# suhrig/arriba

Measured on AMD Instinct MI355X. Metric: chimeric reads/s end-to-end (BAM->fusions.tsv), synthetic, higher is better.
Workload: dtype int32

## Files before the change

arriba_amd/csrc/device/agpu_ingest.hip:

```cpp
#include <hip/hip_runtime.h>
#include <algorithm>
#include <cstring>
#include <string>
#include <vector>
#include <rocprim/rocprim.hpp>
#include "agpu_context.hpp"
#include "ingest_core.hpp"
#include "device_utils.hpp"
#include "shard_host.hpp"
#include "crc32_core.hpp"
#include "inflate_fast_core.hpp"

using namespace agpu;
namespace agpu { extern thread_local bool g_inside_ingest_finish; }

namespace {

const int BLOCK = 256;
inline unsigned int grid_for(uint64_t n, int block = BLOCK) { return (unsigned int) ((n + block - 1) / block); }

enum { IC_ACTIVE = 0, IC_MAPPED_READS = 1, IC_MISSING_HI = 2, IC_BROKEN = 3, IC_MALFORMED = 4, IC_CHIMERIC = 5, IC_COLLISION = 6, IC_MISMATCH = 7, IC_UNSORTED = 8, IC_MAX_NAME = 9,
       IC_MAX_READ_LENGTH = 10, IC_STRAND_COUNT = 11, IC_STRAND_MATCHING = 12, IC_RUNS_UNSORTED = 13, IC_QNAME_COMMA = 14, IC_COUNT = 16 };

#define HIP_CHECK(call) do { hipError_t e_ = (call); if (e_ != hipSuccess) { set_last_error(std::string(#call) + ": " + hipGetErrorString(e_)); return AGPU_ERR_DEVICE; } } while (0)
#define ALLOC(buffer, bytes) do { if (!(buffer).allocate(bytes)) { set_last_error("hipMalloc failed (" #buffer ")"); return AGPU_ERR_NO_MEMORY; } } while (0)
#define TRY(call) do { int s_ = (call); if (s_ != AGPU_OK) return s_; } while (0)


__global__ void __launch_bounds__(BLOCK) bgzf_unwrap_kernel(const uint8_t* raw, const agpu_bgzf_block* blocks, uint8_t* stream) {
	const agpu_bgzf_block block = blocks[blockIdx.x];
	const uint8_t* source = raw + block.raw_offset + block.payload_offset;
	uint8_t* target = stream + block.stream_offset;
	const uint32_t size = block.payload_size;
	uint32_t head = (uint32_t) ((4 - ((uintptr_t) target & 3)) & 3);
	if (head > size) head = size;
	if (threadIdx.x < head) target[threadIdx.x] = source[threadIdx.x];
	const uint32_t words = (size - head) / 4;
	for (uint32_t w = threadIdx.x; w < words; w += BLOCK) *(uint32_t*) (target + head + 4 * (size_t) w) = load_u32(source + head + 4 * (size_t) w);
	const uint32_t tail = head + 4 * words;
	if (threadIdx.x < size - tail) target[tail + threadIdx.x] = source[tail + threadIdx.x];
}

template <int LANES> __global__ void __launch_bounds__(LANES) bgzf_inflate_tokens_kernel(const uint8_t* raw, const agpu_bgzf_block* blocks, uint32_t n_blocks, uint8_t* stream, uint8_t* spill,
                                                                                        unsigned long long* notes, uint32_t* note_count, int* status, unsigned int* failures) {
	__shared__ InflateFastTables tables[LANES];
	const uint32_t b = blockIdx.x * LANES + threadIdx.x;
	if (b >= n_blocks) return;
	const agpu_bgzf_block block = blocks[b];
	const bool partial = block.skip != 0 || block.keep != block.isize;
	uint8_t* target = partial ? spill + (b == 0 ? 0 : 65536) : stream + block.stream_offset;
	uint32_t noted = 0;
	const int result = block.isize > 65536 ? (int) INFLATE_OUTPUT_OVERRUN
	                 : inflate_tokens(raw + block.raw_offset + block.payload_offset, block.payload_size, target, block.isize, notes + (size_t) b * INFLATE_MATCH_CAPACITY, INFLATE_MATCH_CAPACITY, noted, tables[threadIdx.x]);
	note_count[b] = noted; status[b] = result;
	if (result != INFLATE_OK && result != INFLATE_RETRY) atomicAdd(failures, 1u);
}

__global__ void __launch_bounds__(BLOCK) bgzf_inflate_resolve_kernel(const agpu_bgzf_block* blocks, uint32_t n_blocks, uint8_t* stream, uint8_t* spill, const unsigned long long* notes, const uint32_t* note_count, const int* status) {
	const uint32_t b = blockIdx.x * (BLOCK / 64) + (threadIdx.x >> 6), lane = threadIdx.x & 63;
	if (b >= n_blocks || status[b] != INFLATE_OK) return;
	const agpu_bgzf_block block = blocks[b];
	const bool partial = block.skip != 0 || block.keep != block.isize;
	uint8_t* target = partial ? spill + (b == 0 ? 0 : 65536) : stream + block.stream_offset;
	const unsigned long long* mine = notes + (size_t) b * INFLATE_MATCH_CAPACITY;
	const uint32_t n = note_count[b];
	for (uint32_t base = 0; base < n; base += 64) {
		const unsigned long long note = base + lane < n ? mine[base + lane] : 0ull;
		const uint32_t position = inflate_note_position(note), length = inflate_note_length(note), distance = inflate_note_distance(note);
		bool pending = base + lane < n;
		while (true) {
			const unsigned long long waiting = __ballot(pending);
			if (waiting == 0) break;
			const uint32_t frontier = (uint32_t) __shfl((int) position, __ffsll((unsigned long long) waiting) - 1);
			if (pending && inflate_match_is_ready(position, length, distance, frontier)) { inflate_copy_match(target, position, length, distance); pending = false; }
			__builtin_amdgcn_fence(__ATOMIC_SEQ_CST, "workgroup");
		}
	}
	if (partial) for (uint32_t k = lane; k < block.keep; k += 64) stream[block.stream_offset + k] = target[block.skip + k];
}

__global__ void __launch_bounds__(64, 3) bgzf_inflate_kernel(const uint8_t* raw, const agpu_bgzf_block* blocks, uint8_t* stream, uint8_t* spill, int* status, int* verdict, unsigned int* failures) {
	__shared__ InflateShared shared;
	if (status != nullptr && status[blockIdx.x] != INFLATE_RETRY) return;
	const agpu_bgzf_block block = blocks[blockIdx.x];
	const bool partial = block.skip != 0 || block.keep != block.isize;
	uint8_t* target = partial ? spill + (blockIdx.x == 0 ? 0 : 65536) : stream + block.stream_offset;
	auto sync = [] () { __syncthreads(); };
	auto broadcast = [] (uint32_t value) { return (uint32_t) __builtin_amdgcn_readfirstlane((int) value); };
	const int result = inflate_block(raw + block.raw_offset + block.payload_offset, block.payload_size, target, block.isize, shared, threadIdx.x, 64u, sync, broadcast);
	if (verdict != nullptr && threadIdx.x == 0) verdict[blockIdx.x] = result;
	if (result != INFLATE_OK) { if (threadIdx.x == 0) atomicAdd(failures, 1u); return; }
	if (partial) {
		__syncthreads();
		for (uint32_t k = threadIdx.x; k < block.keep; k += 64) stream[block.stream_offset + k] = __hip_atomic_load(&target[block.skip + k], __ATOMIC_RELAXED, __HIP_MEMORY_SCOPE_AGENT);
	}
}


__global__ void segment_guess_kernel(const uint8_t* bytes, uint64_t size, uint64_t base, uint64_t segment_begin, uint64_t n_segments, uint32_t n_targets, uint64_t* first, uint64_t* end, uint32_t* count) {
	const uint64_t s = segment_begin + blockIdx.x * (uint64_t) BLOCK + threadIdx.x;
	if (s < n_segments) guess_segment(bytes, size, base, s, n_targets, first, end, count);
}

__global__ void segment_check_kernel(const uint64_t* first, const uint64_t* end, uint64_t segment_begin, uint64_t n_segments, uint8_t* mismatch, uint32_t* mismatches) {
	__shared__ uint32_t block_sum;
	uint32_t mine = 0;
	for (uint64_t s = segment_begin + blockIdx.x * (uint64_t) BLOCK + threadIdx.x; s < n_segments; s += gridDim.x * (uint64_t) BLOCK) {
		const bool bad = s > 0 && first[s] != end[s - 1];
		mismatch[s] = bad;
		mine += bad;
	}
	block_tally(mine, mismatches, &block_sum);
}

__global__ void segment_repair_kernel(const uint8_t* bytes, uint64_t size, uint64_t base, uint64_t segment_begin, uint64_t n_segments, const uint8_t* mismatch, const uint64_t* previous_end, uint64_t* first, uint64_t* end, uint32_t* count) {
	const uint64_t s = segment_begin + blockIdx.x * (uint64_t) BLOCK + threadIdx.x;
	if (s < n_segments) repair_segment_run(bytes, size, base, n_segments, s, mismatch, previous_end, first, end, count);
}

__global__ void segment_emit_kernel(const uint8_t* bytes, uint64_t size, uint64_t base, uint64_t segment_begin, uint64_t n_segments, const uint64_t* first, const uint32_t* record_base, uint64_t* record_offset) {
	const uint64_t s = segment_begin + blockIdx.x * (uint64_t) BLOCK + threadIdx.x;
	if (s >= n_segments) return;
	const uint64_t begin = base + s * SEGMENT_BYTES, segment_end = (begin + SEGMENT_BYTES < size) ? begin + SEGMENT_BYTES : size;
	uint32_t n = 0;
	walk_segment(bytes, size, first[s], segment_end, n, record_offset + record_base[s]);
}


const uint32_t PARSE_WINDOW = 16384;
__global__ void __launch_bounds__(BLOCK) record_parse_kernel(IngestStream in, GenomeView genome, uint64_t seed, uint64_t record_begin, uint64_t* keys, uint8_t* bits, int32_t* hit_index, uint32_t* counters) {
	__shared__ uint32_t sums[4];
	__shared__ __attribute__((aligned(16))) uint8_t staged[BLOCK / 64][PARSE_WINDOW + 64];
	const uint32_t wave = threadIdx.x / 64, lane = threadIdx.x % 64;
	uint8_t* window = staged[wave];
	uint32_t active = 0, mapped = 0, missing = 0, broken = 0;
	for (uint64_t base = record_begin + ((uint64_t) blockIdx.x * (BLOCK / 64) + wave) * 64; base < in.n_records; base += (uint64_t) gridDim.x * BLOCK) {
		const uint64_t r = base + lane;
		const uint64_t piece_begin = in.record_offset[base] & ~15ull, piece_end = base + 64 < in.n_records ? in.record_offset[base + 64] : in.size;
		const bool in_lds = piece_end > piece_begin && piece_end - piece_begin <= PARSE_WINDOW;
		if (in_lds) {
			for (uint64_t at = piece_begin + 16 * lane; at < piece_end; at += 16 * 64) *(uint4*) (window + (at - piece_begin)) = *(const uint4*) (in.bytes + at);
			__builtin_amdgcn_fence(__ATOMIC_RELEASE, "workgroup"); __builtin_amdgcn_wave_barrier(); __builtin_amdgcn_fence(__ATOMIC_ACQUIRE, "workgroup");
		}
		if (r < in.n_records) {
			const uint64_t offset = in.record_offset[r];
			const uint8_t* p = in.bytes + offset;
			uint32_t block_size = load_u32(p);
			if (in_lds && offset + 4 + (uint64_t) block_size <= piece_end && offset + 36 <= piece_end) { p = window + (offset - piece_begin); block_size = load_u32(p); }
			uint64_t key = ~0ull;
			uint8_t status = RECORD_SKIPPED;
			int32_t hit = HIT_INDEX_UNKNOWN;
			if (!record_sizes_ok(p + 4, block_size)) { status = RECORD_BROKEN; ++broken; }
			else {
				const Rec record = load_record_at(in, p);
				if (!((record.flag & BAMF_UNMAP) || ((record.flag & BAMF_PAIRED) && (record.flag & BAMF_MUNMAP)))) {
					const AuxTags tags = scan_aux(record.aux, record.end);
					if (!tags.has_hi && (record.flag & BAMF_SECONDARY)) { status = RECORD_MISSING_HI; ++missing; }
					else if (record.contig < 0) { status = RECORD_BROKEN; ++broken; }
					else {
						status = RECORD_ACTIVE | (tags.has_sa ? RECORD_HAS_SA : 0);
						key = name_key(record, tags.has_hi ? tags.hi : 1, seed);
						hit = hit_index_to_keep(tags);
						++active;
						if (!(record.flag & BAMF_SUPPLEMENTARY) && (genome.contig_bits[record.contig] & CBIT_INTERESTING)) ++mapped;
					}
				}
			}
			keys[r] = key;
			bits[r] = status;
			hit_index[r] = hit;
		}
		__builtin_amdgcn_fence(__ATOMIC_RELEASE, "workgroup"); __builtin_amdgcn_wave_barrier();
	}
	block_tally(active, &counters[IC_ACTIVE], &sums[0]);
	block_tally(mapped, &counters[IC_MAPPED_READS], &sums[1]);
	block_tally(missing, &counters[IC_MISSING_HI], &sums[2]);
	block_tally(broken, &counters[IC_BROKEN], &sums[3]);
}

__global__ void group_head_kernel(const uint64_t* sorted_keys, uint64_t n_active, uint8_t* head) {
	const uint64_t p = blockIdx.x * (uint64_t) BLOCK + threadIdx.x;
	if (p < n_active) head[p] = p == 0 || sorted_keys[p] != sorted_keys[p - 1];
}
__global__ void group_first_flag_kernel(const uint32_t* sorted_records, const uint32_t* group_start, uint32_t n_groups, uint8_t* first_flags) {
	const uint32_t g = blockIdx.x * BLOCK + threadIdx.x;
	if (g < n_groups) first_flags[sorted_records[group_start[g]]] = 1;
}
__global__ void group_rank_kernel(const uint32_t* sorted_records, const uint32_t* group_start, uint32_t n_groups, uint64_t n_active, const uint32_t* stream_rank, uint32_t* group_first, uint32_t* group_begin, uint32_t* group_count) {
	const uint32_t g = blockIdx.x * BLOCK + threadIdx.x;
	if (g >= n_groups) return;
	const uint32_t begin = group_start[g], first = sorted_records[begin], t = stream_rank[first];
	group_first[t] = first; group_begin[t] = begin; group_count[t] = (uint32_t) ((g + 1 < n_groups ? (uint64_t) group_start[g + 1] : n_active) - begin);
}
__global__ void group_names_kernel(IngestStream in, const uint32_t* sorted_records, const uint32_t* group_begin, const uint32_t* group_count, uint32_t first_group, uint32_t n_groups, uint32_t* counters) {
	const uint32_t t = first_group + blockIdx.x * BLOCK + threadIdx.x;
	if (t >= n_groups || group_count[t] < 2) return;
	const uint32_t* records = sorted_records + group_begin[t];
	const Rec a = load_record(in, records[0]);
	const int64_t hit_a = hit_index_of(in, records[0], a);
	for (uint32_t k = 1; k < group_count[t]; ++k) {
		const Rec b = load_record(in, records[k]);
		if (!same_name(a, hit_a, b, hit_index_of(in, records[k], b))) { atomicOr(&counters[IC_COLLISION], 1u); return; }
	}
}


__global__ void window_carry_kernel(uint32_t* record_base, uint64_t segment_begin, uint64_t segment_end, const uint32_t* records_before) {
	const uint64_t s = segment_begin + blockIdx.x * (uint64_t) BLOCK + threadIdx.x;
	if (s <= segment_end) record_base[s] += *records_before;
}
__global__ void window_summary_kernel(const uint32_t* record_base, const uint64_t* end, uint64_t segment_end, uint32_t* records_before, uint32_t* words) {
	*records_before = record_base[segment_end];
	words[1] = record_base[segment_end];
	const uint64_t last_end = end[segment_end - 1];
	words[4] = (uint32_t) last_end; words[5] = (uint32_t) (last_end >> 32);
}
struct RecordIsActive { __host__ __device__ bool operator()(uint8_t bits) const { return (bits & RECORD_STATUS_MASK) == RECORD_ACTIVE; } };
__global__ void run_head_kernel(const uint64_t* keys, const uint32_t* active_records, uint64_t begin, uint64_t end, uint8_t* head) {
	const uint64_t i = begin + blockIdx.x * (uint64_t) BLOCK + threadIdx.x;
	if (i < end) head[i] = i == 0 || keys[active_records[i]] != keys[active_records[i - 1]];
}
__global__ void run_close_kernel(const uint32_t* active_records, const uint32_t* run_begin, uint32_t first_group, uint32_t n_groups, uint32_t n_runs, uint64_t active_total, uint32_t* group_first, uint32_t* group_count) {
	const uint32_t g = first_group + blockIdx.x * BLOCK + threadIdx.x;
	if (g >= n_groups) return;
	const uint32_t begin = run_begin[g];
	group_first[g] = active_records[begin];
	group_count[g] = (uint32_t) ((g + 1 < n_runs ? (uint64_t) run_begin[g + 1] : active_total) - begin);
}
__global__ void run_key_kernel(const uint64_t* keys, const uint32_t* group_first, uint32_t n_groups, uint64_t* out) {
	const uint32_t g = blockIdx.x * BLOCK + threadIdx.x;
	if (g < n_groups) out[g] = keys[group_first[g]];
}
__global__ void run_repeat_kernel(const uint64_t* sorted_keys, uint32_t n_groups, uint32_t* repeats) {
	__shared__ uint32_t block_sum;
	uint32_t mine = 0;
	for (uint64_t g = blockIdx.x * (uint64_t) BLOCK + threadIdx.x; g < n_groups; g += gridDim.x * (uint64_t) BLOCK) mine += g > 0 && sorted_keys[g] == sorted_keys[g - 1];
	block_tally(mine, repeats, &block_sum);
}

struct ViralCounter {
	unsigned long long* counts;
	__device__ void operator()(uint32_t contig) { atomicAdd(&counts[contig], 1ull); }
};

#ifndef AGPU_REPLAY_WAVES
#define AGPU_REPLAY_WAVES 0
#endif
#ifndef AGPU_PACK_WAVES
#define AGPU_PACK_WAVES 0
#endif
#if AGPU_REPLAY_WAVES > 0
#define AGPU_REPLAY_OCCUPANCY __attribute__((amdgpu_waves_per_eu(AGPU_REPLAY_WAVES, AGPU_REPLAY_WAVES)))
#else
#define AGPU_REPLAY_OCCUPANCY
#endif
#if AGPU_PACK_WAVES > 0
#define AGPU_PACK_OCCUPANCY __attribute__((amdgpu_waves_per_eu(AGPU_PACK_WAVES, AGPU_PACK_WAVES)))
#else
#define AGPU_PACK_OCCUPANCY
#endif
template <bool RUNS> __global__ void __launch_bounds__(BLOCK) AGPU_REPLAY_OCCUPANCY group_replay_kernel(IngestContext ctx, const uint32_t* sorted_records, const uint32_t* group_begin, const uint32_t* group_count, uint32_t first_group, uint32_t n_groups,
                                                             FragmentPlan* plain, TandemPlan* itd, uint8_t* valid, FragmentSizes* sizes, unsigned long long* viral_counts, uint32_t* qname_differs, uint32_t* counters) {
	__shared__ uint32_t sums[2];
	GroupTally tally; tally.malformed = 0; tally.chimeric = 0; tally.collision = 0;
	const uint32_t g = first_group + blockIdx.x * BLOCK + threadIdx.x;
	if (g < n_groups) {
		const uint32_t begin = group_begin[g];
		const uint32_t n_records = group_count[g];
		const Rec representative = load_record(ctx.stream, sorted_records[begin]);
		const int64_t hit = hit_index_of(ctx.stream, sorted_records[begin], representative);
		const uint32_t length = qname_length(representative);
		if (RUNS) {
			if (find_byte(representative.name, length, ',') < length) atomicOr(&counters[IC_QNAME_COMMA], 1u);
			if (g == 0) qname_differs[0] = 0;
			else {
				const uint32_t record_before = sorted_records[group_begin[g - 1]];
				const Rec run_before = load_record(ctx.stream, record_before);
				const uint32_t length_before = qname_length(run_before), shorter = length < length_before ? length : length_before, different = first_difference(run_before.name, representative.name, shorter);
				qname_differs[g] = length != length_before || different < shorter;
				bool unsorted;
				if (different < shorter) unsorted = run_before.name[different] > representative.name[different];
				else unsorted = compare_names(fragment_name(run_before, hit_index_of(ctx.stream, record_before, run_before), false, length_before), fragment_name(representative, hit, false, length)) >= 0;
				if (unsorted) atomicOr(&counters[IC_RUNS_UNSORTED], 1u);
			}
		}
		FragmentPlan plain_plan; TandemPlan itd_plan;
		ViralCounter viral = { viral_counts };
		replay_group(ctx, sorted_records + begin, n_records, plain_plan, itd_plan, tally, viral, RUNS ? &representative : nullptr, length, hit);
		if (tally.collision) atomicOr(&counters[IC_COLLISION], 1u);
		Fragment3 fragment;
		AGPU_NOUNROLL for (uint32_t entry = 0; entry < 2; ++entry) {
			const FragmentPlan& plan = entry ? itd_plan.plan : plain_plan;
			bool ok = false;
			if (plan.count > 0) {
				ok = normalize_plan(ctx.stream, plan, entry ? &itd_plan.tandem : nullptr, fragment);
				if (!ok) tally.malformed++;
			}
			valid[2 * (size_t) g + entry] = ok;
			FragmentSizes mine; mine.cigar_words = 0; mine.sequence_bytes = 0; mine.name_length = 0;
			if (ok) { if (entry) itd[g] = itd_plan; else plain[g] = plain_plan; fragment_sizes(fragment, representative, hit, entry, mine, length); }
			sizes[2 * (size_t) g + entry] = mine;
		}
	}
	block_tally(tally.malformed, &counters[IC_MALFORMED], &sums[0]);
	block_tally(tally.chimeric, &counters[IC_CHIMERIC], &sums[1]);
}


__device__ FragmentName name_of(const IngestStream& in, const uint32_t* group_first, uint32_t ref, Rec& storage) {
	storage = load_record(in, group_first[ref >> 1]);
	return fragment_name(storage, hit_index_of(in, group_first[ref >> 1], storage), ref & 1);
}

__global__ void name_order_check_kernel(IngestStream in, const uint32_t* group_first, const uint32_t* order, uint64_t n, uint32_t* counters) {
	__shared__ uint32_t block_max;
	if (threadIdx.x == 0) block_max = 0;
	__syncthreads();
	const uint64_t i = blockIdx.x * (uint64_t) BLOCK + threadIdx.x;
	if (i < n) {
		Rec storage_a, storage_b;
		const FragmentName mine = name_of(in, group_first, order[i], storage_a);
		atomicMax(&block_max, name_length(mine));
		if (i > 0) {
			const FragmentName before = name_of(in, group_first, order[i - 1], storage_b);
			if (compare_names(before, mine) >= 0) atomicOr(&counters[IC_UNSORTED], 1u);
		}
	}
	__syncthreads();
	if (threadIdx.x == 0 && block_max) atomicMax(&counters[IC_MAX_NAME], block_max);
}

__global__ void run_itd_order_kernel(IngestStream in, const uint32_t* group_first, const uint8_t* valid, uint32_t first_group, uint32_t n_groups, uint32_t* counters) {
	const uint32_t g = first_group + blockIdx.x * BLOCK + threadIdx.x;
	if (g >= n_groups || g == 0 || !valid[2 * (size_t) (g - 1) + 1]) return;
	Rec storage_a, storage_b;
	const FragmentName mine = name_of(in, group_first, 2 * g, storage_b);
	const FragmentName before = name_of(in, group_first, 2 * (g - 1) + 1, storage_a);
	if (compare_names(before, mine) >= 0) atomicOr(&counters[IC_RUNS_UNSORTED], 1u);
}

__global__ void name_chunk_kernel(IngestStream in, const uint32_t* group_first, const uint32_t* order, uint64_t n, uint32_t chunk, uint64_t* keys) {
	const uint64_t i = blockIdx.x * (uint64_t) BLOCK + threadIdx.x;
	if (i >= n) return;
	Rec storage;
	keys[i] = name_chunk(name_of(in, group_first, order[i], storage), chunk);
}


__global__ void fragment_layout_kernel(IngestStream in, const uint32_t* group_first, const uint32_t* order, uint64_t n, const FragmentSizes* sizes, const uint32_t* qname_run ,
                                       uint32_t* cigar_words, uint32_t* sequence_bytes, uint32_t* name_lengths, uint32_t* new_group) {
	const uint64_t i = blockIdx.x * (uint64_t) BLOCK + threadIdx.x;
	if (i > n) return;
	if (i == n) { cigar_words[i] = 0; sequence_bytes[i] = 0; name_lengths[i] = 0; return; }
	const uint32_t ref = order[i];
	const FragmentSizes mine = sizes[ref];
	cigar_words[i] = mine.cigar_words; sequence_bytes[i] = mine.sequence_bytes; name_lengths[i] = mine.name_length;
	uint32_t differs = 0;
	if (i > 0 && qname_run != nullptr) differs = qname_run[ref >> 1] != qname_run[order[i - 1] >> 1];
	else if (i > 0) {
		const Rec a = load_record(in, group_first[ref >> 1]), b = load_record(in, group_first[order[i - 1] >> 1]);
		const uint32_t length = qname_length(a);
		differs = length != qname_length(b);
		for (uint32_t k = 0; k < length && !differs; ++k) differs = a.name[k] != b.name[k];
	}
	new_group[i] = differs;
}

__global__ void __launch_bounds__(BLOCK) AGPU_PACK_OCCUPANCY fragment_pack_kernel(IngestStream in, const uint32_t* group_first, const uint32_t* order, uint64_t n, const FragmentPlan* plain, const TandemPlan* itd,
                                                              const uint64_t* cigar_base, const uint64_t* sequence_base, const uint64_t* name_base, const uint32_t* group_id, PackTarget out, uint32_t* counters) {
	__shared__ uint32_t block_max;
	if (threadIdx.x == 0) block_max = 0;
	__syncthreads();
	const uint64_t i = blockIdx.x * (uint64_t) BLOCK + threadIdx.x;
	if (i == n) out.name_offset[n] = name_base[n];
	if (i < n) {
		const uint32_t ref = order[i], g = ref >> 1;
		const bool is_itd = ref & 1;
		Fragment3 f;
		normalize_plan(in, is_itd ? itd[g].plan : plain[g], is_itd ? &itd[g].tandem : nullptr, f);
		Rec storage;
		const FragmentName name = name_of(in, group_first, ref, storage);
		atomicMax(&block_max, write_fragment(in, f, name, i, cigar_base[i], sequence_base[i], name_base[i], group_id[i], out));
	}
	__syncthreads();
	if (threadIdx.x == 0 && block_max) atomicMax(&counters[IC_MAX_READ_LENGTH], block_max);
}

template <bool INFLATED> __global__ void __launch_bounds__(256) bgzf_crc_kernel(const uint8_t* raw, const agpu_bgzf_block* blocks, uint32_t n_blocks, const Crc32Tables* tables, unsigned int* mismatches) {
	__shared__ uint32_t slice[4][256];
	__shared__ uint32_t join[2][4][256];
	__shared__ uint32_t staged[4][CRC32_WAVE_LANES * (CRC32_ROUND_WORDS + 1)];
	for (uint32_t k = threadIdx.x; k < 4 * 256; k += 256) ((uint32_t*) slice)[k] = ((const uint32_t*) tables->slice)[k];
	for (uint32_t k = threadIdx.x; k < 2 * 4 * 256; k += 256) ((uint32_t*) join)[k] = ((const uint32_t*) tables->join)[k];
	const uint32_t wave = threadIdx.x / CRC32_WAVE_LANES, lane = threadIdx.x % CRC32_WAVE_LANES, b = blockIdx.x * 4 + wave;
	agpu_bgzf_block block;
	block.crc32 = 0; block.payload_size = 0; block.raw_offset = 0; block.payload_offset = 0;
	if (b < n_blocks) block = blocks[b];
	if (INFLATED) { block.raw_offset = block.stream_offset; block.payload_offset = 0; block.payload_size = block.isize; }
	const bool checked = b < n_blocks && block.crc32 != 0 && block.payload_size <= CRC32_VIRTUAL;
	const uint8_t* payload = raw + block.raw_offset + block.payload_offset;
	const uint32_t n = block.payload_size;
	uint32_t* mine = staged[wave];
	uint32_t c = 0;
	const bool by_chunks = checked && n >= 4;
	const uint32_t first_word = by_chunks ? (CRC32_VIRTUAL - n) / 4 : CRC32_VIRTUAL / 4;
	for (uint32_t round = 0; round < CRC32_WAVE_CHUNK / 4 / CRC32_ROUND_WORDS; ++round) {
		__syncthreads();
		for (uint32_t item = lane; item < CRC32_WAVE_LANES * CRC32_ROUND_WORDS; item += CRC32_WAVE_LANES) {
			const uint32_t chunk = item / CRC32_ROUND_WORDS, j = item % CRC32_ROUND_WORDS, w = chunk * (CRC32_WAVE_CHUNK / 4) + round * CRC32_ROUND_WORDS + j;
			mine[chunk * (CRC32_ROUND_WORDS + 1) + j] = w >= first_word ? crc32_virtual_word(payload, n, w) : 0u;
		}
		__syncthreads();
		for (uint32_t j = 0; j < CRC32_ROUND_WORDS; ++j) c = crc32_raw_step(slice, c, mine[lane * (CRC32_ROUND_WORDS + 1) + j]);
	}
	__syncthreads();
	mine[lane] = c;
	__syncthreads();
	if (lane % 8 == 0) { for (uint32_t i = 1; i < 8; ++i) c = crc32_apply(join[0], c) ^ mine[lane + i]; }
	__syncthreads();
	if (lane % 8 == 0) mine[lane] = c;
	__syncthreads();
	if (lane == 0 && checked) {
		for (uint32_t g = 1; g < 8; ++g) c = crc32_apply(join[1], c) ^ mine[8 * g];
		c ^= 0xFFFFFFFFu;
		if (n < 4) c = crc32_of_sliced(slice, payload, n);
		if (c != block.crc32) atomicAdd(mismatches, 1u);
	}
}

__global__ void shard_rebase_kernel(uint32_t* out, const uint32_t* in, uint64_t n, uint32_t base, const uint8_t* n_aln, uint32_t slot) {
	const uint64_t i = (uint64_t) blockIdx.x * blockDim.x + threadIdx.x;
	if (i < n) out[i] = in[i] + ((slot >= 3 || slot < n_aln[i]) ? base : 0u);
}
__global__ void shard_rebase_names_kernel(uint64_t* out, const uint64_t* in, uint64_t n, uint64_t base) {
	const uint64_t i = (uint64_t) blockIdx.x * blockDim.x + threadIdx.x;
	if (i < n) out[i] = in[i] + base;
}
__global__ void shard_add_coverage_kernel(uint32_t* windows, uint8_t* starts, uint8_t* ends, const uint32_t* part_windows, const uint8_t* part_starts, const uint8_t* part_ends, uint64_t n) {
	const uint64_t i = (uint64_t) blockIdx.x * blockDim.x + threadIdx.x;
	if (i < n) { windows[i] += part_windows[i]; starts[i] |= part_starts[i]; ends[i] |= part_ends[i]; }
}
__global__ void shard_add_counts_kernel(unsigned long long* counts, const unsigned long long* part, uint32_t n) {
	const uint32_t i = blockIdx.x * blockDim.x + threadIdx.x;
	if (i < n) counts[i] += part[i];
}

__global__ void packed_name_length_kernel(const uint64_t* name_offset, uint64_t n, uint32_t* longest) {
	const uint64_t i = blockIdx.x * (uint64_t) BLOCK + threadIdx.x;
	if (i < n) atomicMax(longest, (uint32_t) (name_offset[i + 1] - name_offset[i]));
}
__global__ void packed_name_chunk_kernel(const char* names, const uint64_t* name_offset, const uint32_t* order, uint64_t n, uint32_t chunk, uint64_t* keys) {
	const uint64_t i = blockIdx.x * (uint64_t) BLOCK + threadIdx.x;
	if (i >= n) return;
	const uint32_t row = order[i]; const uint64_t begin = name_offset[row]; const uint32_t length = (uint32_t) (name_offset[row + 1] - begin);
	uint64_t key = 0;
	for (uint32_t k = 0; k < 8; ++k) { const uint32_t at = 8 * chunk + k; key = key << 8 | (at < length ? (uint8_t) names[begin + at] : 0u); }
	keys[i] = key;
}
__global__ void packed_name_neighbours_kernel(const char* names, const uint64_t* name_offset, const uint32_t* order, uint64_t n, uint32_t* new_group, uint32_t* equal_names) {
	const uint64_t i = blockIdx.x * (uint64_t) BLOCK + threadIdx.x;
	if (i >= n) return;
	if (i == 0) { new_group[0] = 0; return; }
	const uint32_t a = order[i - 1], b = order[i]; const uint64_t begin_a = name_offset[a], begin_b = name_offset[b]; const uint32_t length_a = (uint32_t) (name_offset[a + 1] - begin_a), length_b = (uint32_t) (name_offset[b + 1] - begin_b);
	bool same = length_a == length_b;
	for (uint32_t k = 0; same && k < length_a; ++k) same = names[begin_a + k] == names[begin_b + k];
	if (same) atomicAdd(equal_names, 1u);
	uint32_t qname_a = length_a, qname_b = length_b;
	while (qname_a > 0 && names[begin_a + qname_a - 1] != ',') --qname_a;
	while (qname_b > 0 && names[begin_b + qname_b - 1] != ',') --qname_b;
	bool same_qname = qname_a == qname_b;
	for (uint32_t k = 0; same_qname && k < qname_a; ++k) same_qname = names[begin_a + k] == names[begin_b + k];
	new_group[i] = same_qname ? 0u : 1u;
}
__global__ void qname_run_flag_kernel(IngestStream in, uint64_t n_records, uint8_t* flags) {
	const uint64_t r = blockIdx.x * (uint64_t) BLOCK + threadIdx.x;
	if (r < n_records) flags[r] = starts_qname_run(in, (uint32_t) r) ? 1 : 0;
}
__global__ void qname_key_kernel(IngestStream in, const uint32_t* run_starts, uint64_t n_runs, uint64_t* keys) {
	const uint64_t k = blockIdx.x * (uint64_t) BLOCK + threadIdx.x;
	if (k < n_runs) qname_key128(load_record(in, run_starts[k]), keys[2 * k], keys[2 * k + 1]);
}
__global__ void qname_low_kernel(const uint64_t* keys, uint64_t n, uint64_t* low) { const uint64_t k = blockIdx.x * (uint64_t) BLOCK + threadIdx.x; if (k < n) low[k] = keys[2 * k]; }
__global__ void qname_equal_kernel(const uint64_t* low_sorted, const uint32_t* index_sorted, const uint64_t* keys, uint64_t n, uint32_t* equal) {
	const uint64_t k = blockIdx.x * (uint64_t) BLOCK + threadIdx.x;
	if (k > 0 && k < n && low_sorted[k] == low_sorted[k - 1] && keys[2 * (uint64_t) index_sorted[k] + 1] == keys[2 * (uint64_t) index_sorted[k - 1] + 1]) atomicAdd(equal, 1u);
}
__global__ void iota_kernel(uint32_t* out, uint64_t n) { const uint64_t i = blockIdx.x * (uint64_t) BLOCK + threadIdx.x; if (i < n) out[i] = (uint32_t) i; }

__global__ void coverage_from_differences_kernel(const uint32_t* summed, const uint64_t* window_offset, uint32_t n_contigs, uint64_t n, uint32_t* counts, uint16_t* out) {
	const uint64_t i = blockIdx.x * (uint64_t) BLOCK + threadIdx.x;
	if (i >= n) return;
	uint32_t low = 0, high = n_contigs;
	while (high - low > 1) { const uint32_t middle = (low + high) / 2; if (window_offset[middle] <= i) low = middle; else high = middle; }
	const uint32_t count = summed[i + low];
	counts[i] = count;
	out[i] = count > 65535u ? (uint16_t) 65535 : (uint16_t) count;
}
__global__ void coverage_clamp_kernel(const uint32_t* windows, uint64_t n, uint16_t* out) {
	const uint64_t i = blockIdx.x * (uint64_t) BLOCK + threadIdx.x;
	if (i < n) out[i] = windows[i] > 65535u ? (uint16_t) 65535 : (uint16_t) windows[i];
}


__global__ void gather_sizes_kernel(BatchView b, const uint64_t* name_offset, const uint32_t* ids, uint64_t n, uint32_t* cigar_words, uint32_t* sequence_bytes, uint32_t* name_lengths) {
	const uint64_t k = blockIdx.x * (uint64_t) BLOCK + threadIdx.x;
	if (k > n) return;
	if (k == n) { cigar_words[k] = 0; sequence_bytes[k] = 0; name_lengths[k] = 0; return; }
	row_sizes(b, name_offset, ids ? ids[k] : k, cigar_words[k], sequence_bytes[k], name_lengths[k]);
}

__global__ void gather_copy_kernel(BatchView b, const uint8_t* pristine_fbits, const uint8_t* const* pristine_abits, const uint64_t* name_offset, const char* names, const uint32_t* ids, uint64_t n,
                                   const uint64_t* cigar_base, const uint64_t* sequence_base, const uint64_t* name_base, PackTarget out) {
	const uint64_t k = blockIdx.x * (uint64_t) BLOCK + threadIdx.x;
	if (k == n) { if (out.name_offset) out.name_offset[n] = name_base[n]; else out.row_name_offset[n] = (uint32_t) name_base[n]; }
	if (k >= n) return;
	copy_row(b, pristine_fbits, pristine_abits, name_offset, names, ids ? ids[k] : k, k, cigar_base[k], sequence_base[k], name_base[k], out);
}


__global__ void strandedness_flag_kernel(BatchView b, AnnotationView ann, uint64_t first, uint64_t count, uint8_t* flags) {
	const uint64_t k = blockIdx.x * (uint64_t) BLOCK + threadIdx.x;
	if (k >= count) return;
	flags[k] = strandedness_vote(b, ann, first + k);
}

__global__ void strandedness_take_kernel(const uint8_t* flags, uint64_t count, uint32_t wanted, uint32_t* counters) {
	if (blockIdx.x != 0 || threadIdx.x != 0) return;
	uint32_t seen = counters[IC_STRAND_COUNT], matching = counters[IC_STRAND_MATCHING];
	for (uint64_t k = 0; k < count && seen < wanted; ++k)
		if (flags[k]) { ++seen; if (flags[k] & 2) ++matching; }
	counters[IC_STRAND_COUNT] = seen; counters[IC_STRAND_MATCHING] = matching;
}


int grow_stream(agpu_ctx* ctx, uint64_t needed) {
	needed += 64;
	if (needed <= ctx->ingest_stream.capacity) { ctx->ingest_stream.bytes = needed; return AGPU_OK; }
	DeviceBuffer larger;
	const uint64_t doubled = ctx->ingest_stream.capacity * 2;
	if (!larger.allocate(std::max<uint64_t>(needed + (needed >> 3), std::max<uint64_t>(doubled, 64u << 20)))) { set_last_error("hipMalloc failed (BAM stream)"); return AGPU_ERR_NO_MEMORY; }
	if (ctx->piece_stream) { HIP_CHECK(hipStreamSynchronize(ctx->piece_stream)); HIP_CHECK(hipStreamSynchronize(ctx->piece_stream2)); }
	if (ctx->ingest_stream_size > 0) HIP_CHECK(hipMemcpyAsync(larger.ptr, ctx->ingest_stream.ptr, ctx->ingest_stream_size, hipMemcpyDeviceToDevice, ctx->stream));
	HIP_CHECK(hipStreamSynchronize(ctx->stream));
	if (ctx->ingest_progress.work) HIP_CHECK(hipStreamSynchronize(ctx->ingest_progress.work));
	ctx->ingest_stream.swap(larger);
	return AGPU_OK;
}

int wait_for_previous_push(agpu_ctx* ctx) {
	const uint32_t behind = ctx->ingest_host_buffers - 1;
	if (ctx->ingest_pushes >= behind) HIP_CHECK(hipEventSynchronize(ctx->piece_copied[(ctx->ingest_pushes - behind) % AGPU_PIECE_SLOTS]));
	return AGPU_OK;
}

template <class Key> int sort_pairs(agpu_ctx* ctx, DeviceBuffer& scratch, Key* keys_in, Key* keys_out, uint32_t* values_in, uint32_t* values_out, uint64_t n, unsigned int end_bit, const char* label, bool counting_values) {
	size_t bytes = 0;
	hipStream_t s = ctx->stream;
	if (counting_values) HIP_CHECK(rocprim::radix_sort_pairs(nullptr, bytes, keys_in, keys_out, rocprim::counting_iterator<uint32_t>(0), values_out, n, 0, end_bit, s));
	else HIP_CHECK(rocprim::radix_sort_pairs(nullptr, bytes, keys_in, keys_out, values_in, values_out, n, 0, end_bit, s));
	if (bytes > scratch.capacity) ALLOC(scratch, bytes);
	KernelTimer timer(ctx, label, n * (uint64_t) (sizeof(Key) + 4) * 2);
	if (counting_values) HIP_CHECK(rocprim::radix_sort_pairs(scratch.ptr, bytes, keys_in, keys_out, rocprim::counting_iterator<uint32_t>(0), values_out, n, 0, end_bit, s));
	else HIP_CHECK(rocprim::radix_sort_pairs(scratch.ptr, bytes, keys_in, keys_out, values_in, values_out, n, 0, end_bit, s));
	return AGPU_OK;
}

int select_flagged(agpu_ctx* ctx, DeviceBuffer& scratch, const uint8_t* flags, uint32_t* out, uint32_t* device_count, uint64_t n) {
	size_t bytes = 0;
	HIP_CHECK(rocprim::select(nullptr, bytes, rocprim::counting_iterator<uint32_t>(0), flags, out, device_count, n, ctx->stream));
	if (bytes > scratch.capacity) ALLOC(scratch, bytes);
	HIP_CHECK(rocprim::select(scratch.ptr, bytes, rocprim::counting_iterator<uint32_t>(0), flags, out, device_count, n, ctx->stream));
	return AGPU_OK;
}

int exclusive_sum_u64(agpu_ctx* ctx, DeviceBuffer& scratch, const uint32_t* in, uint64_t* out, uint64_t n) {
	size_t bytes = 0;
	HIP_CHECK(rocprim::exclusive_scan(nullptr, bytes, in, out, (uint64_t) 0, n, rocprim::plus<uint64_t>(), ctx->stream));
	if (bytes > scratch.capacity) ALLOC(scratch, bytes);
	HIP_CHECK(rocprim::exclusive_scan(scratch.ptr, bytes, in, out, (uint64_t) 0, n, rocprim::plus<uint64_t>(), ctx->stream));
	return AGPU_OK;
}


const unsigned int INGEST_WINDOW_RING = 16, INGEST_WINDOW_WORDS = 8;
uint64_t g_window_bytes = 512u << 20;
uint64_t g_window_margin = 1u << 20;

int grow_keeping(agpu_ctx* ctx, DeviceBuffer& buffer, size_t needed, size_t used, size_t estimate) {
	if (needed == 0) needed = 16;
	if (buffer.ptr != nullptr && needed <= buffer.capacity) { if (needed > buffer.bytes) buffer.bytes = needed; return AGPU_OK; }
	DeviceBuffer larger;
	if (!larger.allocate(std::max(needed + needed / 2, estimate)) && !larger.allocate(needed)) { set_last_error("hipMalloc failed (tables of the ingest)"); return AGPU_ERR_NO_MEMORY; }
	hipStream_t s = ctx->ingest_progress.work;
	if (used > 0 && buffer.ptr != nullptr) HIP_CHECK(hipMemcpyAsync(larger.ptr, buffer.ptr, std::min(used, buffer.capacity), hipMemcpyDeviceToDevice, s));
	HIP_CHECK(hipStreamSynchronize(s));
	buffer.swap(larger);
	return AGPU_OK;
}

IngestStream window_stream(agpu_ctx* ctx, uint64_t size, uint64_t n_records) {
	IngestStream in;
	in.bytes = ctx->ingest_stream.as<uint8_t>(); in.size = size; in.record_offset = ctx->scratch("ingest.record_offset").as<uint64_t>(); in.n_records = n_records;
	in.n_targets = ctx->ingest_n_targets; in.tid_to_contig = ctx->ingest_tid_to_contig.as<uint32_t>();
	in.hit_index = ctx->scratch("ingest.hit_index").as<int32_t>();
	return in;
}

IngestContext replay_context(agpu_ctx* ctx, const IngestStream& in) {
	IngestContext context;
	context.stream = in; context.annotation = ctx->annotation; context.annotation.n_dummy = 0; context.genome = ctx->genome;
	context.coverage.n_contigs = ctx->genome.n_contigs; context.coverage.window_offset = ctx->coverage_window_offset.as<uint64_t>(); context.coverage.windows = ctx->coverage_windows32.as<uint32_t>();
	context.coverage.fragment_starts = ctx->coverage_fragment_starts.as<uint8_t>(); context.coverage.fragment_ends = ctx->coverage_fragment_ends.as<uint8_t>();
	if (getenv("ARRIBA_INGEST_SKIP_COVERAGE") != nullptr) context.coverage.windows = nullptr;
	context.record_bits = ctx->scratch("ingest.record_bits").as<uint8_t>(); context.max_itd_length = ctx->ingest_max_itd_length; context.external_duplicate_marking = ctx->ingest_external_duplicate_marking;
	return context;
}

int window_step(agpu_ctx* ctx, IngestWindow& w) {
	IngestProgress& p = ctx->ingest_progress;
	hipStream_t s = p.work;
	uint32_t* words = ctx->scratch("ingest.window_words").as<uint32_t>() + (size_t) w.slot * INGEST_WINDOW_WORDS;
	uint32_t* device_counters = ctx->scratch("ingest.counters").as<uint32_t>();
	DeviceBuffer& rocprim_scratch = ctx->scratch("ingest.window_rocprim");
	const uint64_t base = ctx->ingest_first_record;
	const uint8_t* bytes = ctx->ingest_stream.as<uint8_t>();
	const uint64_t n = w.segment_end - w.segment_begin;
	const size_t estimated_records = (size_t) (p.size_hint / 128 + 4096);
	size_t temporary = 0;
	switch (w.enqueued + 1) {
	case 1: {
		HIP_CHECK(hipMemsetAsync(words, 0, INGEST_WINDOW_WORDS * 4, s));
		if (n == 0) break;
		DeviceBuffer& first = ctx->scratch("ingest.segment_first"); DeviceBuffer& end = ctx->scratch("ingest.segment_end"); DeviceBuffer& end_before = ctx->scratch("ingest.segment_end_before");
		DeviceBuffer& count = ctx->scratch("ingest.segment_count"); DeviceBuffer& record_base = ctx->scratch("ingest.segment_base"); DeviceBuffer& mismatch = ctx->scratch("ingest.segment_mismatch");
		const size_t segments = (size_t) w.segment_end + 1, done = (size_t) w.segment_begin + 1, estimate = (size_t) (p.size_hint / SEGMENT_BYTES + 16);
		TRY(grow_keeping(ctx, first, segments * 8, done * 8, estimate * 8)); TRY(grow_keeping(ctx, end, segments * 8, done * 8, estimate * 8)); TRY(grow_keeping(ctx, end_before, segments * 8, 0, estimate * 8));
		TRY(grow_keeping(ctx, count, segments * 4, done * 4, estimate * 4)); TRY(grow_keeping(ctx, record_base, segments * 4, done * 4, estimate * 4)); TRY(grow_keeping(ctx, mismatch, segments, done, estimate));
		{ KernelTimer timer(ctx, "segment_guess_kernel", n * SEGMENT_BYTES, s);
		  segment_guess_kernel<<<grid_for(n), BLOCK, 0, s>>>(bytes, w.avail, base, w.segment_begin, w.segment_end, ctx->ingest_n_targets, first.as<uint64_t>(), end.as<uint64_t>(), count.as<uint32_t>()); }
		for (int pass = 0; pass < 3; ++pass) {
			segment_check_kernel<<<tally_grid(n, BLOCK), BLOCK, 0, s>>>(first.as<uint64_t>(), end.as<uint64_t>(), w.segment_begin, w.segment_end, mismatch.as<uint8_t>(), words + 6);
			const uint64_t from = w.segment_begin > 0 ? w.segment_begin - 1 : 0;
			HIP_CHECK(hipMemcpyAsync(end_before.as<uint64_t>() + from, end.as<uint64_t>() + from, (w.segment_end - from) * 8, hipMemcpyDeviceToDevice, s));
			segment_repair_kernel<<<grid_for(n), BLOCK, 0, s>>>(bytes, w.avail, base, w.segment_begin, w.segment_end, mismatch.as<uint8_t>(), end_before.as<uint64_t>(), first.as<uint64_t>(), end.as<uint64_t>(), count.as<uint32_t>());
		}
		segment_check_kernel<<<tally_grid(n, BLOCK), BLOCK, 0, s>>>(first.as<uint64_t>(), end.as<uint64_t>(), w.segment_begin, w.segment_end, mismatch.as<uint8_t>(), words + 0);
		HIP_CHECK(hipMemsetAsync(count.as<uint32_t>() + w.segment_end, 0, 4, s));
		HIP_CHECK(rocprim::exclusive_scan(nullptr, temporary, count.as<uint32_t>() + w.segment_begin, record_base.as<uint32_t>() + w.segment_begin, 0u, n + 1, rocprim::plus<uint32_t>(), s));
		if (temporary > rocprim_scratch.capacity) ALLOC(rocprim_scratch, temporary);
		HIP_CHECK(rocprim::exclusive_scan(rocprim_scratch.ptr, temporary, count.as<uint32_t>() + w.segment_begin, record_base.as<uint32_t>() + w.segment_begin, 0u, n + 1, rocprim::plus<uint32_t>(), s));
		uint32_t* records_before = ctx->scratch("ingest.window_state").as<uint32_t>();
		window_carry_kernel<<<grid_for(n + 1), BLOCK, 0, s>>>(record_base.as<uint32_t>(), w.segment_begin, w.segment_end, records_before);
		window_summary_kernel<<<1, 1, 0, s>>>(record_base.as<uint32_t>(), end.as<uint64_t>(), w.segment_end, records_before, words);
		break; }
	case 2: {
		const uint64_t records = w.record_end - w.record_begin;
		w.active_begin = p.active;
		if (records == 0) break;
		DeviceBuffer& record_offset = ctx->scratch("ingest.record_offset"); DeviceBuffer& keys = ctx->scratch("ingest.keys"); DeviceBuffer& record_bits = ctx->scratch("ingest.record_bits"); DeviceBuffer& active_records = ctx->scratch("ingest.sorted_records");
		TRY(grow_keeping(ctx, record_offset, w.record_end * 8, w.record_begin * 8, estimated_records * 8)); TRY(grow_keeping(ctx, keys, w.record_end * 8, w.record_begin * 8, estimated_records * 8));
		TRY(grow_keeping(ctx, ctx->scratch("ingest.hit_index"), w.record_end * 4, w.record_begin * 4, estimated_records * 4));
		TRY(grow_keeping(ctx, record_bits, w.record_end, w.record_begin, estimated_records)); TRY(grow_keeping(ctx, active_records, (w.active_begin + records) * 4, w.active_begin * 4, estimated_records * 4));
		{ KernelTimer timer(ctx, "segment_emit_kernel", records * 8, s);
		  segment_emit_kernel<<<grid_for(n), BLOCK, 0, s>>>(bytes, w.avail, base, w.segment_begin, w.segment_end, ctx->scratch("ingest.segment_first").as<uint64_t>(), ctx->scratch("ingest.segment_base").as<uint32_t>(), record_offset.as<uint64_t>()); }
		const IngestStream in = window_stream(ctx, w.avail, w.record_end);
		{ KernelTimer timer(ctx, "record_parse_kernel", records * (8 + 64 + 9), s);
		  record_parse_kernel<<<tally_grid(records, BLOCK) * 8, BLOCK, 0, s>>>(in, ctx->genome, 0, w.record_begin, keys.as<uint64_t>(), record_bits.as<uint8_t>(), ctx->scratch("ingest.hit_index").as<int32_t>(), device_counters); }
		auto flags = rocprim::make_transform_iterator(record_bits.as<uint8_t>() + w.record_begin, RecordIsActive());
		HIP_CHECK(rocprim::select(nullptr, temporary, rocprim::counting_iterator<uint32_t>((uint32_t) w.record_begin), flags, active_records.as<uint32_t>() + w.active_begin, words + 2, records, s));
		if (temporary > rocprim_scratch.capacity) ALLOC(rocprim_scratch, temporary);
		HIP_CHECK(rocprim::select(rocprim_scratch.ptr, temporary, rocprim::counting_iterator<uint32_t>((uint32_t) w.record_begin), flags, active_records.as<uint32_t>() + w.active_begin, words + 2, records, s));
		break; }
	case 3: {
		const uint64_t active = w.active_end - w.active_begin;
		w.head_begin = p.heads;
		if (active == 0) break;
		DeviceBuffer& head = ctx->scratch("ingest.head"); DeviceBuffer& run_begin = ctx->scratch("ingest.group_begin");
		TRY(grow_keeping(ctx, head, w.active_end, 0, estimated_records)); TRY(grow_keeping(ctx, run_begin, (w.head_begin + active + 1) * 4, w.head_begin * 4, estimated_records * 2));
		{ KernelTimer timer(ctx, "run_head_kernel", active * (8 + 4 + 1), s);
		  run_head_kernel<<<grid_for(active), BLOCK, 0, s>>>(ctx->scratch("ingest.keys").as<uint64_t>(), ctx->scratch("ingest.sorted_records").as<uint32_t>(), w.active_begin, w.active_end, head.as<uint8_t>()); }
		HIP_CHECK(rocprim::select(nullptr, temporary, rocprim::counting_iterator<uint32_t>((uint32_t) w.active_begin), head.as<uint8_t>() + w.active_begin, run_begin.as<uint32_t>() + w.head_begin, words + 3, active, s));
		if (temporary > rocprim_scratch.capacity) ALLOC(rocprim_scratch, temporary);
		HIP_CHECK(rocprim::select(rocprim_scratch.ptr, temporary, rocprim::counting_iterator<uint32_t>((uint32_t) w.active_begin), head.as<uint8_t>() + w.active_begin, run_begin.as<uint32_t>() + w.head_begin, words + 3, active, s));
		break; }
	case 4: {
// ... 1161 lines not shown
```

arriba_amd/csrc/device/ingest_core.hpp:

```cpp
#ifndef AGPU_INGEST_CORE_HPP
#define AGPU_INGEST_CORE_HPP 1

#include "annotate_core.hpp"
#include "event_core.hpp"

namespace agpu {


AGPU_HD uint32_t load_u32(const uint8_t* p) { uint32_t v; __builtin_memcpy(&v, p, 4); return v; }
AGPU_HD uint64_t load_u64(const uint8_t* p) { uint64_t v; __builtin_memcpy(&v, p, 8); return v; }
AGPU_HD uint32_t first_zero_byte(uint64_t v) { const uint64_t z = (v - 0x0101010101010101ull) & ~v & 0x8080808080808080ull; return z ? (uint32_t) __builtin_ctzll(z) >> 3 : 8u; }
AGPU_HD uint64_t low_bytes(uint32_t n) { return n >= 8 ? ~0ull : (1ull << (8 * n)) - 1; }
AGPU_HD uint32_t find_byte(const uint8_t* p, uint32_t n, uint8_t byte) {
	const uint64_t pattern = 0x0101010101010101ull * byte;
	uint32_t i = 0;
	for (; i + 8 <= n; i += 8) { const uint32_t z = first_zero_byte(load_u64(p + i) ^ pattern); if (z < 8) return i + z; }
	if (i == n) return n;
	if (n >= 8) {
		const uint32_t z = first_zero_byte((load_u64(p + n - 8) ^ pattern) | low_bytes(i - (n - 8)));
		return z < 8 ? n - 8 + z : n;
	}
	for (; i < n; ++i) if (p[i] == byte) return i;
	return n;
}
AGPU_HD uint32_t first_difference(const uint8_t* a, const uint8_t* b, uint32_t n) {
	uint32_t i = 0;
	for (; i + 8 <= n; i += 8) { const uint64_t x = load_u64(a + i) ^ load_u64(b + i); if (x) return i + ((uint32_t) __builtin_ctzll(x) >> 3); }
	if (i == n) return n;
	if (n >= 8) {
		const uint64_t x = (load_u64(a + n - 8) ^ load_u64(b + n - 8)) & ~low_bytes(i - (n - 8));
		return x ? n - 8 + ((uint32_t) __builtin_ctzll(x) >> 3) : n;
	}
	for (; i < n; ++i) if (a[i] != b[i]) return i;
	return n;
}
AGPU_HD uint16_t load_u16(const uint8_t* p) { uint16_t v; __builtin_memcpy(&v, p, 2); return v; }

enum : uint16_t { BAMF_PAIRED = 1, BAMF_PROPER_PAIR = 2, BAMF_UNMAP = 4, BAMF_MUNMAP = 8, BAMF_REVERSE = 16, BAMF_READ1 = 64, BAMF_SECONDARY = 256, BAMF_DUP = 1024, BAMF_SUPPLEMENTARY = 2048 };

AGPU_HD bool op_consumes_query(uint32_t op) { return (0x3C1A7u >> (op << 1)) & 1; }
AGPU_HD bool op_consumes_reference(uint32_t op) { return (0x3C1A7u >> (op << 1)) & 2; }

struct IngestStream {
	const uint8_t* bytes;
	uint64_t size;
	const uint64_t* record_offset;
	uint64_t n_records;
	uint32_t n_targets;
	const uint32_t* tid_to_contig;
	const int32_t* hit_index;
};
const int32_t HIT_INDEX_UNKNOWN = -0x7FFFFFFF - 1;

struct Rec {
	const uint8_t* cigar_bytes; const uint8_t* seq_bytes; const uint8_t* name; const uint8_t* aux; const uint8_t* end;
	int32_t contig, pos, l_seq;
	uint32_t n_cigar, l_read_name;
	uint16_t flag;
	AGPU_HD uint32_t cigar(uint32_t i) const { return load_u32(cigar_bytes + 4 * (size_t) i); }
	AGPU_HD uint32_t op(uint32_t i) const { return cigar(i) & 15; }
	AGPU_HD uint32_t len(uint32_t i) const { return cigar(i) >> 4; }
	AGPU_HD uint32_t code(int32_t i) const { return (seq_bytes[i >> 1] >> ((~i & 1) << 2)) & 15; }
	AGPU_HD bool forward() const { return !(flag & BAMF_REVERSE); }
	AGPU_HD bool paired() const { return flag & BAMF_PAIRED; }
	AGPU_HD int32_t qlen(uint32_t n) const { int32_t l = 0; for (uint32_t i = 0; i < n; ++i) if (op_consumes_query(op(i))) l += (int32_t) len(i); return l; }
	AGPU_HD int32_t rlen(uint32_t n) const { int32_t l = 0; for (uint32_t i = 0; i < n; ++i) if (op_consumes_reference(op(i))) l += (int32_t) len(i); return l; }
	AGPU_HD int32_t endpos() const { int32_t l = (!(flag & BAMF_UNMAP) && n_cigar > 0) ? rlen(n_cigar) : 1; return pos + (l == 0 ? 1 : l); }
};

AGPU_HD bool record_sizes_ok(const uint8_t* block, uint32_t block_size) {
	if (block_size < 32) return false;
	const uint32_t l_read_name = block[8], n_cigar = load_u16(block + 12);
	const int32_t l_seq = (int32_t) load_u32(block + 16);
	if (l_seq < 0 || l_read_name == 0) return false;
	const uint64_t fixed = 32ull + l_read_name + 4ull * n_cigar + ((uint64_t) l_seq + 1) / 2 + (uint64_t) l_seq;
	return fixed <= block_size;
}

AGPU_HD Rec load_record_at(const IngestStream& in, const uint8_t* p) {
	const uint64_t word0 = load_u64(p), word1 = load_u64(p + 8), word2 = load_u64(p + 16);
	const uint32_t block_size = (uint32_t) word0;
	p += 4;
	Rec rec;
	const int32_t tid = (int32_t) (word0 >> 32);
	rec.contig = (tid >= 0 && (uint32_t) tid < in.n_targets) ? (int32_t) in.tid_to_contig[tid] : -1;
	rec.pos = (int32_t) (uint32_t) word1;
	rec.l_read_name = (uint32_t) (word1 >> 32) & 0xFFu;
	rec.n_cigar = (uint32_t) word2 & 0xFFFFu;
	rec.flag = (uint16_t) (word2 >> 16);
	rec.l_seq = (int32_t) (word2 >> 32);
	rec.name = p + 32;
	rec.cigar_bytes = rec.name + rec.l_read_name;
	rec.seq_bytes = rec.cigar_bytes + 4 * (size_t) rec.n_cigar;
	rec.aux = rec.seq_bytes + ((size_t) rec.l_seq + 1) / 2 + (size_t) rec.l_seq;
	rec.end = p + block_size;
	return rec;
}
AGPU_HD Rec load_record(const IngestStream& in, uint32_t r) { return load_record_at(in, in.bytes + in.record_offset[r]); }


const uint32_t SEGMENT_BYTES = 8192;
const uint64_t SEARCH_LIMIT = 4u << 20;
const uint64_t OFFSET_NONE = ~0ull, OFFSET_BROKEN = ~0ull - 1;

AGPU_HD bool plausible_record(const uint8_t* bytes, uint64_t size, uint64_t o, uint32_t n_targets) {
	if (o + 36 > size) return false;
	const uint32_t block_size = load_u32(bytes + o);
	if (block_size < 32 || block_size > (1u << 28) || o + 4 + (uint64_t) block_size > size) return false;
	const uint8_t* p = bytes + o + 4;
	const int32_t tid = (int32_t) load_u32(p), pos = (int32_t) load_u32(p + 4), next_tid = (int32_t) load_u32(p + 20), next_pos = (int32_t) load_u32(p + 24);
	if (tid < -1 || tid >= (int32_t) n_targets || next_tid < -1 || next_tid >= (int32_t) n_targets || pos < -1 || next_pos < -1) return false;
	if (!record_sizes_ok(p, block_size)) return false;
	const uint32_t l_read_name = p[8];
	return p[32 + l_read_name - 1] == 0;
}

AGPU_HD uint64_t walk_segment(const uint8_t* bytes, uint64_t size, uint64_t start, uint64_t segment_end, uint32_t& count, uint64_t* offsets) {
	uint64_t o = start;
	count = 0;
	while (o < segment_end) {
		if (o + 4 > size) return OFFSET_BROKEN;
		const uint32_t block_size = load_u32(bytes + o);
		if (block_size < 32 || o + 4 + (uint64_t) block_size > size) return OFFSET_BROKEN;
		if (offsets != nullptr) offsets[count] = o;
		++count;
		o += 4 + (uint64_t) block_size;
	}
	return o;
}

AGPU_HD void guess_segment(const uint8_t* bytes, uint64_t size, uint64_t base, uint64_t s, uint32_t n_targets, uint64_t* first, uint64_t* end, uint32_t* count) {
	const uint64_t begin = base + s * SEGMENT_BYTES, segment_end = (begin + SEGMENT_BYTES < size) ? begin + SEGMENT_BYTES : size;
	uint64_t start = OFFSET_NONE;
	if (s == 0) start = base;
	else {
		const uint64_t limit = (begin + SEARCH_LIMIT < size) ? begin + SEARCH_LIMIT : size;
		for (uint64_t o = begin; o < limit; ++o) {
			if (!plausible_record(bytes, size, o, n_targets)) continue;
			const uint64_t next = o + 4 + (uint64_t) load_u32(bytes + o);
			if (next == size || plausible_record(bytes, size, next, n_targets)) { start = o; break; }
		}
	}
	first[s] = start;
	uint32_t n = 0;
	end[s] = (start == OFFSET_NONE) ? OFFSET_NONE : walk_segment(bytes, size, start, segment_end, n, nullptr);
	count[s] = n;
}

AGPU_HD void repair_segment_run(const uint8_t* bytes, uint64_t size, uint64_t base, uint64_t n_segments, uint64_t s, const uint8_t* mismatch, const uint64_t* previous_end, uint64_t* first, uint64_t* end, uint32_t* count) {
	if (!mismatch[s] || mismatch[s - 1]) return;
	uint64_t start = previous_end[s - 1];
	for (uint64_t t = s; t < n_segments && (t == s || mismatch[t]); ++t) {
		const uint64_t begin = base + t * SEGMENT_BYTES, segment_end = (begin + SEGMENT_BYTES < size) ? begin + SEGMENT_BYTES : size;
		first[t] = start;
		uint32_t n = 0;
		end[t] = (start >= OFFSET_BROKEN) ? start : walk_segment(bytes, size, start, segment_end, n, nullptr);
		count[t] = n;
		start = end[t];
	}
}

struct AuxTags { bool has_hi, has_sa; int64_t hi; };
AGPU_HD AuxTags scan_aux(const uint8_t* s, const uint8_t* end) {
	AuxTags tags; tags.has_hi = false; tags.has_sa = false; tags.hi = 0;
	while (s + 3 <= end) {
		const uint8_t* value = s + 2;
		size_t size;
		switch (*value) {
			case 'A': case 'c': case 'C': size = 2; break;
			case 's': case 'S': size = 3; break;
			case 'i': case 'I': case 'f': size = 5; break;
			case 'd': size = 9; break;
			case 'Z': case 'H': { const uint8_t* p = value + 1; while (p < end && *p) ++p; if (p >= end) return tags; size = (size_t) (p - value) + 1; break; }
			case 'B': {
				if (value + 6 > end) return tags;
				const size_t element = (value[1] == 'c' || value[1] == 'C') ? 1 : (value[1] == 's' || value[1] == 'S') ? 2 : 4;
				size = 6 + element * (size_t) load_u32(value + 2);
				break;
			}
			default: return tags;
		}
		if (value + size > end) return tags;
		if (s[0] == 'H' && s[1] == 'I' && !tags.has_hi) {
			tags.has_hi = true;
			switch (*value) {
				case 'c': tags.hi = (int8_t) value[1]; break;
				case 'C': tags.hi = value[1]; break;
				case 's': tags.hi = (int16_t) load_u16(value + 1); break;
				case 'S': tags.hi = load_u16(value + 1); break;
				case 'i': tags.hi = (int32_t) load_u32(value + 1); break;
				case 'I': tags.hi = load_u32(value + 1); break;
				default: tags.hi = 0; break;
			}
		}
		if (s[0] == 'S' && s[1] == 'A') tags.has_sa = true;
		if (tags.has_hi && tags.has_sa) return tags;
		s = value + size;
	}
	return tags;
}

AGPU_HD int32_t hit_index_to_keep(const AuxTags& tags) { const int64_t hi = tags.has_hi ? tags.hi : 1; return (hi > HIT_INDEX_UNKNOWN && hi <= 0x7FFFFFFF) ? (int32_t) hi : HIT_INDEX_UNKNOWN; }
AGPU_HD int64_t hit_index_of(const IngestStream& in, uint32_t record, const Rec& rec) {
	if (in.hit_index != nullptr) { const int32_t kept = in.hit_index[record]; if (kept != HIT_INDEX_UNKNOWN) return kept; }
	const AuxTags tags = scan_aux(rec.aux, rec.end);
	return tags.has_hi ? tags.hi : 1;
}

enum : uint8_t { RECORD_SKIPPED = 0, RECORD_ACTIVE = 1, RECORD_MISSING_HI = 2, RECORD_BROKEN = 3, RECORD_STATUS_MASK = 3, RECORD_HAS_SA = 4 };

AGPU_HD uint32_t qname_length(const Rec& r) { return find_byte(r.name, r.l_read_name, 0); }

AGPU_HD bool starts_qname_run(const IngestStream& in, uint32_t record) {
	if (record == 0) return true;
	const Rec a = load_record(in, record - 1), b = load_record(in, record);
	const uint32_t length = qname_length(b);
	if (qname_length(a) != length) return true;
	for (uint32_t i = 0; i < length; ++i) if (a.name[i] != b.name[i]) return true;
	return false;
}
AGPU_HD void qname_key128(const Rec& r, uint64_t& low, uint64_t& high) {
	uint64_t h = 1469598103934665603ull, g = 0x9AE16A3B2F90404Full;
	for (uint32_t i = 0; i < r.l_read_name && r.name[i]; ++i) { h = (h ^ r.name[i]) * 1099511628211ull; g = (g ^ (r.name[i] + 0x9Eu)) * 0x100000001B3ull; g ^= g >> 29; }
	h ^= h >> 33; h *= 0xFF51AFD7ED558CCDull; h ^= h >> 33; h *= 0xC4CEB9FE1A85EC53ull; h ^= h >> 33;
	g ^= g >> 31; g *= 0x7FB5D329728EA185ull; g ^= g >> 27; g *= 0x81DADEF4BC2DD44Dull; g ^= g >> 33;
	low = h; high = g;
}

AGPU_HD uint64_t name_key(const Rec& r, int64_t hit_index, uint64_t seed) {
	uint64_t h = 1469598103934665603ull ^ seed;
	for (uint32_t i = 0; i < r.l_read_name && r.name[i]; ++i) h = (h ^ r.name[i]) * 1099511628211ull;
	h ^= (uint64_t) hit_index * 0x9E3779B97F4A7C15ull;
	h ^= h >> 33; h *= 0xFF51AFD7ED558CCDull; h ^= h >> 33; h *= 0xC4CEB9FE1A85EC53ull; h ^= h >> 33;
	return h == ~0ull ? ~0ull - 1 : h;
}
AGPU_HD bool same_name(const Rec& a, uint32_t length_a , int64_t hi_a, const Rec& b, int64_t hi_b) {
	if (hi_a != hi_b) return false;
	if (length_a != qname_length(b)) return false;
	return first_difference(a.name, b.name, length_a) == length_a;
}
AGPU_HD bool same_name(const Rec& a, int64_t hi_a, const Rec& b, int64_t hi_b) { return same_name(a, qname_length(a), hi_a, b, hi_b); }


enum : uint8_t { CLIP_NONE = 0, CLIP_START = 1, CLIP_END = 2, PLAN_TANDEM = 3 };
const uint32_t NO_RECORD = 0xFFFFFFFFu;

struct PlanEntry { uint32_t record; uint16_t cigar_index; uint8_t clip; uint8_t supplementary; };
struct TandemAlignment { int32_t start, end; uint32_t cigar[3]; uint32_t record; uint8_t n_cigar, strand, first_in_pair, supplementary; };
struct FragmentPlan {
	PlanEntry entry[3];
	uint8_t count;
	uint8_t single_end, duplicate, reserved;
};
struct TandemPlan { FragmentPlan plan; TandemAlignment tandem; };

AGPU_HD void plan_clear(FragmentPlan& plan) { plan.count = 0; plan.single_end = 0; plan.duplicate = 0; plan.reserved = 0; for (int k = 0; k < 3; ++k) { plan.entry[k].record = NO_RECORD; plan.entry[k].cigar_index = 0; plan.entry[k].clip = 0; plan.entry[k].supplementary = 0; } }
AGPU_HD void plan_push(FragmentPlan& plan, uint32_t record, const Rec& r, bool is_supplementary, uint32_t cigar_index, uint8_t clip) {
	plan.single_end = !(r.flag & BAMF_PAIRED);
	plan.duplicate = plan.duplicate || (r.flag & BAMF_DUP);
	if (plan.count < 3) {
		PlanEntry& e = plan.entry[plan.count];
		e.record = record; e.cigar_index = (uint16_t) cigar_index; e.clip = clip; e.supplementary = is_supplementary;
	}
	if (plan.count < 255) ++plan.count;
}
AGPU_HD void plan_push_tandem(FragmentPlan& plan) {
	if (plan.count < 3) { PlanEntry& e = plan.entry[plan.count]; e.record = NO_RECORD; e.cigar_index = 0; e.clip = PLAN_TANDEM; e.supplementary = 0; }
	if (plan.count < 255) ++plan.count;
}

struct Aln {
	const uint8_t* cigar_bytes;
	uint32_t record;
	uint32_t sequence_record;
	int32_t sequence_length;
	int32_t contig, start, end;
	uint32_t n_cigar;
	uint32_t cigar_index;
	uint32_t patch_index[2], patch_value[2];
	uint32_t tandem_cigar[3];
	uint32_t made_index, made_value, shift;
	uint8_t clip, n_patch;
	bool supplementary, first_in_pair, strand;
	AGPU_HD uint32_t base_cigar(uint32_t i) const {
		if (clip == PLAN_TANDEM) return i == 0 ? tandem_cigar[0] : i == 1 ? tandem_cigar[1] : tandem_cigar[2];
		if (i == made_index) return made_value;
		return load_u32(cigar_bytes + 4 * (size_t) (i + shift));
	}
	AGPU_HD uint32_t cigar(uint32_t i) const {
		uint32_t value = base_cigar(i);
		for (uint32_t k = 0; k < n_patch; ++k) if (patch_index[k] == i) value = patch_value[k];
		return value;
	}
	AGPU_HD void set_cigar(uint32_t i, uint32_t value) {
		for (uint32_t k = 0; k < n_patch; ++k) if (patch_index[k] == i) { patch_value[k] = value; return; }
		if (n_patch < 2) { patch_index[n_patch] = i; patch_value[n_patch] = value; ++n_patch; }
	}
	AGPU_HD uint32_t preclipping() const { const uint32_t c = cigar(0), op = c & 15; return (op == CIGAR_S || op == CIGAR_H) ? c >> 4 : 0; }
	AGPU_HD uint32_t postclipping() const { const uint32_t c = cigar(n_cigar - 1), op = c & 15; return (op == CIGAR_S || op == CIGAR_H) ? c >> 4 : 0; }
};

AGPU_HD Aln materialize(const IngestStream& in, const PlanEntry& e, const TandemAlignment* tandem) {
	Aln a;
	a.n_patch = 0; a.patch_index[0] = a.patch_index[1] = 0; a.patch_value[0] = a.patch_value[1] = 0;
	a.tandem_cigar[0] = a.tandem_cigar[1] = a.tandem_cigar[2] = 0;
	a.clip = e.clip; a.cigar_index = e.cigar_index;
	a.made_index = NO_RECORD; a.made_value = 0; a.shift = 0;
	if (e.clip == PLAN_TANDEM) {
		const Rec source = load_record(in, tandem->record);
		a.cigar_bytes = source.cigar_bytes;
		a.record = NO_RECORD;
		a.supplementary = tandem->supplementary; a.first_in_pair = tandem->first_in_pair; a.strand = tandem->strand;
		a.contig = source.contig; a.start = tandem->start; a.end = tandem->end;
		a.n_cigar = tandem->n_cigar;
		for (int k = 0; k < 3; ++k) a.tandem_cigar[k] = tandem->cigar[k];
		a.sequence_record = a.supplementary ? NO_RECORD : tandem->record;
		a.sequence_length = a.supplementary ? 0 : source.l_seq;
		return a;
	}
	const Rec r = load_record(in, e.record);
	a.cigar_bytes = r.cigar_bytes;
	a.record = e.record;
	a.strand = r.forward(); a.first_in_pair = r.flag & BAMF_READ1; a.contig = r.contig; a.supplementary = e.supplementary;
	a.sequence_record = e.supplementary ? NO_RECORD : e.record;
	a.sequence_length = e.supplementary ? 0 : r.l_seq;
	if (e.clip == CLIP_START) {
		a.start = r.pos + r.rlen(e.cigar_index); a.end = r.endpos() - 1;
		a.n_cigar = r.n_cigar - e.cigar_index + 1;
		a.made_index = 0; a.made_value = (uint32_t) r.qlen(e.cigar_index) << 4 | (r.op(0) == CIGAR_H ? CIGAR_H : CIGAR_S);
		a.shift = (uint32_t) e.cigar_index - 1u;
	} else if (e.clip == CLIP_END) {
		a.start = r.pos; a.end = r.pos + r.rlen((uint32_t) e.cigar_index + 1) - 1;
		a.n_cigar = (uint32_t) e.cigar_index + 2;
		a.made_index = (uint32_t) e.cigar_index + 1; a.made_value = (uint32_t) (r.l_seq - r.qlen((uint32_t) e.cigar_index + 1)) << 4 | (r.op(r.n_cigar - 1) == CIGAR_H ? CIGAR_H : CIGAR_S);
	} else {
		a.start = r.pos; a.end = r.endpos() - 1;
		a.n_cigar = r.n_cigar;
	}
	return a;
}


AGPU_HD bool is_clipped_at_correct_end(const Rec& r) {
	if (!(r.flag & BAMF_PAIRED)) return true;
	if (r.n_cigar == 0) return false;
	uint32_t clipped_end;
	if (r.flag & BAMF_SUPPLEMENTARY) clipped_end = r.forward() ? r.n_cigar - 1 : 0;
	else clipped_end = r.forward() ? 0 : r.n_cigar - 1;
	const uint32_t op = r.op(clipped_end);
	return op == CIGAR_S || op == CIGAR_H;
}

AGPU_HD bool is_pristine_alignment(const Rec& r) {
	for (uint32_t i = 0; i < r.n_cigar; ++i) {
		const uint32_t op = r.op(i);
		if (op != CIGAR_N && op != CIGAR_M && op != CIGAR_X) return false;
	}
	const uint32_t size = (uint32_t) r.l_seq;
	for (uint32_t i = 2, repeat = 0, count = 1; i + 2 < size; i += 2) {
		if (r.code(i) == r.code(repeat) && r.code(i + 1) == r.code(repeat + 1)) {
			count++;
		} else if (r.code(i + 1) == r.code(repeat + 1) && r.code(i + 2) == r.code(repeat + 2)) {
			count++;
			i++;
		} else {
			count = 1;
			repeat = i;
		}
		if (count >= 8) return false;
	}
	return true;
}

AGPU_HD bool clipped_sequence_is_adapter(const Rec& mate1, const Rec* mate2) {
	if (mate2 == nullptr) return false;
	if (mate1.pos == mate2->pos && mate1.n_cigar > 0 && mate2->n_cigar > 0) {
		if (!mate1.forward() && mate1.op(0) == CIGAR_S && mate2->forward() && mate2->op(mate2->n_cigar - 1) == CIGAR_S && mate1.len(0) == mate2->len(mate2->n_cigar - 1)) return true;
		if (!mate2->forward() && mate2->op(0) == CIGAR_S && mate1.forward() && mate1.op(mate1.n_cigar - 1) == CIGAR_S && mate2->len(0) == mate1.len(mate1.n_cigar - 1)) return true;
	}
	return false;
}

AGPU_HD char base_character(uint32_t code) {
	const uint64_t low = 0x565352474D43413Dull , high = 0x4E42444B48595754ull ;
	return (char) (((code & 8) ? high : low) >> (8 * (code & 7)));
}
AGPU_HD uint32_t nonzero_bytes(uint64_t x) {
	const uint64_t high = (x | ((x & 0x7F7F7F7F7F7F7F7Full) + 0x7F7F7F7F7F7F7F7Full)) & 0x8080808080808080ull;
	return (uint32_t) (((high >> 7) * 0x0102040810204080ull) >> 56);
}

AGPU_HD bool is_tandem_duplication(const Rec* r, uint32_t record, const GenomeView& genome, const uint32_t max_itd_length, TandemAlignment& tandem) {
	const unsigned int min_clipped_length = 12, min_duplication_length = 9, max_duplication_length = max_itd_length;
	const unsigned int max_mismatches = 1, max_non_template_bases = 6, min_alignment_length = 15;
	if (r == nullptr || r->n_cigar == 0) return false;
	unsigned int clipped_length = 0, clipped_position = 0;
	bool clipped_start = true;
	int direction = +1, window_start = 0, window_end = 0, extended_read_start = 0;
	if (r->op(0) == CIGAR_S && r->len(0) >= min_clipped_length) {
		clipped_length = r->len(0);
		clipped_position = 0;
		direction = -1;
		window_start = r->pos + min_duplication_length - clipped_length;
		window_end = r->pos + max_duplication_length - clipped_length;
		extended_read_start = r->pos - clipped_length;
		clipped_start = true;
	}
	if (r->op(r->n_cigar - 1) == CIGAR_S && r->len(r->n_cigar - 1) >= (min_clipped_length > clipped_length ? min_clipped_length : clipped_length)) {
		clipped_length = r->len(r->n_cigar - 1);
		clipped_position = r->l_seq - clipped_length;
		direction = +1;
		window_start = r->endpos() - max_duplication_length;
		window_end = r->endpos() - min_duplication_length;
		extended_read_start = r->endpos();
		clipped_start = false;
	}
	if (clipped_length == 0) return false;
	if (r->contig < 0 || (uint32_t) r->contig >= genome.n_contigs) return false;
	const uint64_t contig_begin = genome.contig_offset[r->contig];
	const uint64_t contig_size = genome.contig_offset[r->contig + 1] - contig_begin;
	if (contig_size == 0) return false;
	const char* contig_sequence = genome.bases + contig_begin;
	if ((uint64_t) (unsigned int) (window_end + max_duplication_length + clipped_length + 1) >= contig_size ||
	    window_start <= (int) (max_duplication_length + clipped_length + 1))
		return false;

	const float min_extended_align_fraction = 0.7;
	unsigned int extended_matches = 0;
	for (unsigned int read_pos = 0; read_pos < clipped_length; ++read_pos)
		if ((uint64_t) (unsigned int) (extended_read_start + read_pos) < contig_size)
			if (contig_sequence[(unsigned int) (extended_read_start + read_pos)] == base_character(r->code((int32_t) (clipped_position + read_pos))))
				extended_matches++;
	if (1.0 * extended_matches / clipped_length >= min_extended_align_fraction) return false;

	const unsigned int held = clipped_length < 16 ? clipped_length : 16;
	uint64_t read_low = 0, read_high = 0;
	for (unsigned int i = 0; i < held; ++i) {
		const int read_pos = (direction == +1) ? (int) i : (int) (clipped_length - 1 - i);
		const uint64_t character = (uint8_t) base_character(r->code((int32_t) clipped_position + read_pos));
		if (i < 8) read_low |= character << (8 * i); else read_high |= character << (8 * (i - 8));
	}
	const uint32_t held_bits = (1u << held) - 1;
	for (int contig_pos = window_start; contig_pos <= window_end; ++contig_pos) {
		if (max_mismatches == 1 && max_non_template_bases == 6) {
			uint64_t contig_low, contig_high;
			if (direction == +1) { contig_low = load_u64((const uint8_t*) contig_sequence + contig_pos); contig_high = load_u64((const uint8_t*) contig_sequence + contig_pos + 8); }
			else {
				const uint8_t* last = (const uint8_t*) contig_sequence + contig_pos + (int) clipped_length - 1;
				contig_low = __builtin_bswap64(load_u64(last - 7)); contig_high = __builtin_bswap64(load_u64(last - 15));
			}
			const uint32_t differs = (nonzero_bytes(contig_low ^ read_low) | nonzero_bytes(contig_high ^ read_high) << 8) & held_bits;
			const uint32_t counted = differs & ~0x3Fu, second = counted & (counted - 1);
			if (second != 0) {
				const uint32_t at = (uint32_t) __builtin_ctz(second);
				if ((uint32_t) __builtin_popcount(~differs & ((1u << at) - 1)) + 2 != clipped_length) continue;
			}
		}
		unsigned int matches = 0, mismatches = 0;
		int tandem_start = (int) contig_size, tandem_end = -1;
		for (unsigned int i = 0; i < clipped_length; i++) {
			const int read_pos = (direction == +1) ? (int) i : (int) (clipped_length - 1 - i);
			if (contig_sequence[contig_pos + read_pos] == base_character(r->code((int32_t) clipped_position + read_pos))) {
				matches++;
				if (contig_pos + read_pos < tandem_start) tandem_start = contig_pos + read_pos;
				if (contig_pos + read_pos > tandem_end) tandem_end = contig_pos + read_pos;
			} else if (i >= max_non_template_bases) {
				mismatches++;
				if (mismatches > max_mismatches) break;
			}
		}
		if (matches >= min_alignment_length || matches + mismatches == clipped_length) {
			tandem.start = tandem_start; tandem.end = tandem_end;
			tandem.record = record;
			tandem.strand = r->forward();
			tandem.first_in_pair = (r->flag & BAMF_READ1) != 0;
			tandem.supplementary = !(r->flag & BAMF_PAIRED) || (clipped_start && r->forward()) || (!clipped_start && !r->forward());
			uint32_t clip_left = clipped_start ? 0 : r->l_seq - clipped_length;
			uint32_t clip_right = clipped_start ? r->l_seq - clipped_length : 0;
			if (tandem_start > contig_pos) clip_left += tandem_start - contig_pos;
			if (tandem_end < contig_pos + (int) clipped_length - 1) clip_right += contig_pos + clipped_length - 1 - tandem_end;
			tandem.n_cigar = 0;
			tandem.cigar[0] = tandem.cigar[1] = tandem.cigar[2] = 0;
			if (clip_left > 0) tandem.cigar[tandem.n_cigar++] = clip_left << 4 | CIGAR_S;
			tandem.cigar[tandem.n_cigar++] = (uint32_t) (tandem_end - tandem_start + 1) << 4 | CIGAR_M;
			if (clip_right > 0) tandem.cigar[tandem.n_cigar++] = clip_right << 4 | CIGAR_S;
			return true;
		}
	}
	return false;
}

AGPU_HD bool find_spanning_intron(const Rec& r, int32_t gene1_end, int32_t gene2_start, uint32_t& cigar_index, int32_t& read_pos) {
	if (r.n_cigar < 3) return false;
	int32_t before = r.pos, after;
	for (uint32_t i = 0; i < r.n_cigar; ++i) {
		const uint32_t op = r.op(i);
		const uint32_t op_length = op_consumes_reference(op) ? r.len(i) : 0;
		after = before + (int32_t) op_length;
		if (op == CIGAR_N && ((before <= gene1_end && after > gene1_end) || (before < gene2_start && after >= gene2_start))) {
			cigar_index = i;
			read_pos = r.qlen(i);
			return true;
		}
		before = after;
	}
	return false;
}

AGPU_HD ListRef genes_at(const FlatIndexView& gene_index, int32_t contig, int32_t position) {
	if (contig < 0 || (uint32_t) contig >= gene_index.n_contigs) return empty_list();
	const uint32_t k = index_lower_bound(gene_index, (uint32_t) contig, position);
	if (k == gene_index.contig_offset[contig + 1]) return empty_list();
	return index_bucket(gene_index, k);
}
AGPU_HD bool lists_intersect(ListRef a, ListRef b) {
	uint32_t i = 0, j = 0;
	while (i < a.n && j < b.n) { const uint32_t x = a.p[i], y = b.p[j]; if (x < y) ++i; else if (y < x) ++j; else return true; }
	return false;
}
AGPU_HD void boundaries_of_biggest_gene(const AnnotationView& ann, ListRef genes, int32_t& start, int32_t& end) {
	start = -1; end = -1;
	for (uint32_t g = 0; g < genes.n; ++g) {
		const int32_t gene_start = ann.gene_start[genes.p[g]], gene_end = ann.gene_end[genes.p[g]];
		if (start == -1 || start > gene_start) start = gene_start;
		if (end == -1 || end < gene_end) end = gene_end;
	}
}

AGPU_HD bool extract_read_through_alignment(FragmentPlan& plan, uint32_t record_index, const Rec& record, uint32_t previous_index, const Rec* previous, const AnnotationView& ann) {
	const Rec* forward_mate = &record; const Rec* reverse_mate = previous;
	uint32_t forward_index = record_index, reverse_index = previous_index;
	if (!forward_mate->forward()) { const Rec* t = forward_mate; forward_mate = reverse_mate; reverse_mate = t; const uint32_t ti = forward_index; forward_index = reverse_index; reverse_index = ti; }
	ListRef forward_genes, reverse_genes;
	if (forward_mate != nullptr) forward_genes = genes_at(ann.gene_index, forward_mate->contig, forward_mate->pos);
	else forward_genes = genes_at(ann.gene_index, reverse_mate->contig, reverse_mate->pos);
	if (reverse_mate != nullptr) reverse_genes = genes_at(ann.gene_index, reverse_mate->contig, reverse_mate->endpos());
	else reverse_genes = genes_at(ann.gene_index, forward_mate->contig, forward_mate->endpos());
	const bool common_empty = !lists_intersect(forward_genes, reverse_genes);
	if (!(common_empty && !(forward_genes.n == 0 && reverse_genes.n == 0))) return false;

	int32_t forward_gene_start, forward_gene_end, reverse_gene_start, reverse_gene_end;
	boundaries_of_biggest_gene(ann, forward_genes, forward_gene_start, forward_gene_end);
	boundaries_of_biggest_gene(ann, reverse_genes, reverse_gene_start, reverse_gene_end);
	if (forward_gene_end == -1) forward_gene_end = reverse_gene_start - 1;
	if (reverse_gene_start == -1) reverse_gene_start = forward_gene_end + 1;

	uint32_t forward_cigar_op = 0, reverse_cigar_op = 0;
	int32_t forward_read_pos = 0, reverse_read_pos = 0;
	const bool forward_has_intron = (forward_mate == nullptr) ? false : find_spanning_intron(*forward_mate, forward_gene_end, reverse_gene_start, forward_cigar_op, forward_read_pos);
	const bool reverse_has_intron = (reverse_mate == nullptr) ? false : find_spanning_intron(*reverse_mate, forward_gene_end, reverse_gene_start, reverse_cigar_op, reverse_read_pos);
	const bool is_new = plan.count == 0;
	if (forward_has_intron && (!reverse_has_intron || forward_read_pos < reverse_mate->l_seq - reverse_read_pos)) {
		if (is_new) {
			plan_push(plan, forward_index, *forward_mate, false, forward_cigar_op + 1, CLIP_START);
			plan_push(plan, forward_index, *forward_mate, true, forward_cigar_op - 1, CLIP_END);
			if (reverse_mate != nullptr) {
				if (reverse_has_intron) plan_push(plan, reverse_index, *reverse_mate, false, reverse_cigar_op + 1, CLIP_START);
				else plan_push(plan, reverse_index, *reverse_mate, false, 0, CLIP_NONE);
			}
			return true;
		}
	} else if (reverse_has_intron) {
		if (is_new) {
			plan_push(plan, reverse_index, *reverse_mate, true, reverse_cigar_op + 1, CLIP_START);
			plan_push(plan, reverse_index, *reverse_mate, false, reverse_cigar_op - 1, CLIP_END);
			if (forward_mate != nullptr) {
				if (forward_has_intron) plan_push(plan, forward_index, *forward_mate, false, forward_cigar_op - 1, CLIP_END);
				else plan_push(plan, forward_index, *forward_mate, false, 0, CLIP_NONE);
			}
			return true;
		}
	} else if (forward_mate != nullptr && reverse_mate != nullptr && reverse_mate->pos >= reverse_gene_start && forward_mate->endpos() <= forward_gene_end) {
		if (is_new) {
			plan_push(plan, forward_index, *forward_mate, false, 0, CLIP_NONE);
			plan_push(plan, reverse_index, *reverse_mate, false, 0, CLIP_NONE);
		}
		return true;
	}
	return false;
}


struct CoverageBuild {
	uint32_t n_contigs;
	const uint64_t* window_offset;
	uint32_t* windows;
	uint8_t* fragment_starts;
	uint8_t* fragment_ends;
};
AGPU_HD uint64_t coverage_difference_slots(uint64_t windows, uint32_t n_contigs) { return windows + n_contigs; }

AGPU_HD void coverage_add(uint32_t* slot, uint32_t value) {
#if defined(__HIP_DEVICE_COMPILE__)
	__hip_atomic_fetch_add(slot, value, __ATOMIC_RELAXED, __HIP_MEMORY_SCOPE_AGENT);
#else
	__atomic_fetch_add(slot, value, __ATOMIC_RELAXED);
#endif
}
struct CoverageRange {
	uint64_t base; int64_t lo, hi;
	AGPU_HD void flush(uint32_t* differences) { if (hi > lo) { coverage_add(&differences[base + (uint64_t) lo], 1u); coverage_add(&differences[base + (uint64_t) hi], 0xFFFFFFFFu); } hi = lo = 0; }
	AGPU_HD void add(uint32_t* differences, uint64_t to_base, int64_t from, int64_t to) {
		if (hi > lo && to_base == base && from == hi) { hi = to; return; }
		flush(differences);
		base = to_base; lo = from; hi = to;
	}
};

AGPU_HD void add_fragment_to_coverage(const CoverageBuild& coverage, const Rec& mate1, uint16_t flag1, const Rec* mate2_or_null, bool is_chimeric) {
	const Rec& mate2 = (mate2_or_null == nullptr) ? mate1 : *mate2_or_null;
	if (coverage.windows == nullptr) return;
	if (mate1.contig < 0 || (uint32_t) mate1.contig >= coverage.n_contigs || mate2.contig < 0 || (uint32_t) mate2.contig >= coverage.n_contigs) return;
	const uint64_t begin1 = coverage.window_offset[mate1.contig], size1 = coverage.window_offset[mate1.contig + 1] - begin1;
	const uint64_t begin2 = coverage.window_offset[mate2.contig], size2 = coverage.window_offset[mate2.contig + 1] - begin2;
	if (size1 == 0 || size2 == 0) return;
	if ((flag1 & BAMF_PAIRED) && !(flag1 & BAMF_PROPER_PAIR)) is_chimeric = true;
	if (!is_chimeric) {
		if (!(flag1 & BAMF_REVERSE) || !(flag1 & BAMF_PAIRED)) { const uint64_t w = (uint64_t) (mate1.pos / COVERAGE_RESOLUTION); if (mate1.pos >= 0 && w < size1) coverage.fragment_starts[begin1 + w] = 1; }
		else { const uint64_t w = (uint64_t) (mate2.pos / COVERAGE_RESOLUTION); if (mate2.pos >= 0 && w < size2) coverage.fragment_starts[begin2 + w] = 1; }
	}
	int32_t position1 = mate1.pos, position2 = mate2.pos;
	int32_t position = position1 < position2 ? position1 : position2;
	int32_t window = position / COVERAGE_RESOLUTION;
	uint32_t i1 = 0, i2 = 0;
	const uint64_t slots1 = begin1 + (uint64_t) mate1.contig, slots2 = begin2 + (uint64_t) mate2.contig;
	CoverageRange pending; pending.base = 0; pending.lo = pending.hi = 0;
	while (true) {
		uint32_t op1 = 0, op2 = 0, length1, length2;
		if (i1 < mate1.n_cigar) { op1 = mate1.cigar(i1); length1 = op_consumes_reference(op1 & 15) ? op1 >> 4 : 0; }
		else { length1 = 0; if (position2 / COVERAGE_RESOLUTION > window) window = position2 / COVERAGE_RESOLUTION; }
		if (i2 < mate2.n_cigar) { op2 = mate2.cigar(i2); length2 = op_consumes_reference(op2 & 15) ? op2 >> 4 : 0; }
		else { length2 = 0; if (position1 / COVERAGE_RESOLUTION > window) window = position1 / COVERAGE_RESOLUTION; }
		uint32_t op;
		uint64_t begin, size;
		if (i1 < mate1.n_cigar && (position1 + (int32_t) length1 < position2 + (int32_t) length2 || i2 >= mate2.n_cigar)) {
			i1++;
			if (length1 == 0) continue;
			op = op1; begin = slots1; size = size1; position1 += (int32_t) length1; position = position1;
		} else if (i2 < mate2.n_cigar) {
			i2++;
			if (length2 == 0) continue;
			op = op2; begin = slots2; size = size2; position2 += (int32_t) length2; position = position2;
		} else {
			break;
		}
		if (op_consumes_query(op & 15)) {
			const int32_t last = position / COVERAGE_RESOLUTION;
			if (window <= last) {
				if (position >= 0) {
					const int64_t from = window > 0 ? window : 0;
					int64_t to = (position - last * COVERAGE_RESOLUTION >= COVERAGE_RESOLUTION / 2) ? (int64_t) last + 1 : (int64_t) last;
					if (to > (int64_t) size) to = (int64_t) size;
					if (to > from) pending.add(coverage.windows, begin, from, to);
				}
				window = last + 1;
			}
		} else {
			window = position / COVERAGE_RESOLUTION;
		}
	}
	pending.flush(coverage.windows);
	if (!is_chimeric) {
		if ((flag1 & BAMF_REVERSE) || !(flag1 & BAMF_PAIRED)) { const uint64_t w = (uint64_t) ((position1 - 1) / COVERAGE_RESOLUTION); if (position1 >= 1 && w < size1) coverage.fragment_ends[begin1 + w] = 1; }
		else { const uint64_t w = (uint64_t) ((position2 - 1) / COVERAGE_RESOLUTION); if (position2 >= 1 && w < size2) coverage.fragment_ends[begin2 + w] = 1; }
	}
}


struct IngestContext {
	IngestStream stream;
	AnnotationView annotation;
	GenomeView genome;
	CoverageBuild coverage;
	const uint8_t* record_bits;
	uint32_t max_itd_length;
	uint8_t external_duplicate_marking;
};

struct GroupTally { uint32_t malformed; uint32_t chimeric; uint32_t collision; };

template <class ViralCounter> AGPU_HD void replay_group(const IngestContext& ctx, const uint32_t* records, uint32_t n_records, FragmentPlan& plain, TandemPlan& itd, GroupTally& tally, ViralCounter& count_viral_read,
                                                        const Rec* names_of = nullptr, uint32_t length_of_names = 0 , int64_t hit_index_of_names = 0) {
	plan_clear(plain); plan_clear(itd.plan);
	itd.tandem.start = 0; itd.tandem.end = 0; itd.tandem.cigar[0] = itd.tandem.cigar[1] = itd.tandem.cigar[2] = 0; itd.tandem.record = NO_RECORD;
	itd.tandem.n_cigar = 0; itd.tandem.strand = 0; itd.tandem.first_in_pair = 0; itd.tandem.supplementary = 0;
	uint32_t parked = NO_RECORD;
	for (uint32_t k = 0; k < n_records; ++k) {
		const uint32_t index = records[k];
		const Rec record = load_record(ctx.stream, index);
		if (names_of != nullptr && k > 0 && !same_name(*names_of, length_of_names, hit_index_of_names, record, hit_index_of(ctx.stream, index, record))) tally.collision = 1;
		if (record.flag & BAMF_SUPPLEMENTARY) {
			if (is_clipped_at_correct_end(record)) plan_push(plain, index, record, true, 0, CLIP_NONE);
			else tally.malformed++;
			tally.chimeric = 1;
			continue;
		}
		uint32_t previous_index = NO_RECORD;
		Rec previous_storage;
		const Rec* previous = nullptr;
		bool is_read_through = false;
		uint16_t coverage_flag = record.flag;
		const bool discordant_mate = (record.flag & BAMF_PAIRED) && !(record.flag & BAMF_PROPER_PAIR);
		if (discordant_mate) {
			plan_push(plain, index, record, false, 0, CLIP_NONE);
			tally.chimeric = 1;
			coverage_flag = 0; is_read_through = true;
		} else {
			if (record.flag & BAMF_PAIRED) {
				if (parked == NO_RECORD) { parked = index; continue; }
				previous_index = parked; parked = NO_RECORD;
				previous_storage = load_record(ctx.stream, previous_index);
				previous = &previous_storage;
			}
			bool is_tandem_alignment = false;
			if (!clipped_sequence_is_adapter(record, previous) && (previous == nullptr || record.forward() != previous->forward())) {
				TandemAlignment tandem;
				bool found = false;
				AGPU_NOUNROLL for (uint32_t mate = 0; mate < 2 && !found; ++mate) found = is_tandem_duplication(mate ? previous : &record, mate ? previous_index : index, ctx.genome, ctx.max_itd_length, tandem);
				if (found) {
					plan_push(itd.plan, index, record, record.forward() == (bool) tandem.strand && !tandem.supplementary, 0, CLIP_NONE);
					if (previous != nullptr) plan_push(itd.plan, previous_index, *previous, previous->forward() == (bool) tandem.strand && !tandem.supplementary, 0, CLIP_NONE);
					if (itd.plan.count < 3) itd.tandem = tandem;
					plan_push_tandem(itd.plan);
					is_tandem_alignment = true;
				}
			}
			const bool record_has_sa = ctx.record_bits[index] & RECORD_HAS_SA, previous_has_sa = previous != nullptr && (ctx.record_bits[previous_index] & RECORD_HAS_SA);
			if ((record_has_sa && is_clipped_at_correct_end(record)) || (previous_has_sa && is_clipped_at_correct_end(*previous))) {
				plan_push(plain, index, record, false, 0, CLIP_NONE);
				if (previous != nullptr) plan_push(plain, previous_index, *previous, false, 0, CLIP_NONE);
				tally.chimeric = 1;
			} else if (!is_tandem_alignment) {
				is_read_through = extract_read_through_alignment(plain, index, record, previous_index, previous, ctx.annotation);
				if (record.contig >= 0 && (ctx.genome.contig_bits[record.contig] & CBIT_VIRAL)) {
					AGPU_NOUNROLL for (uint32_t mate = 0; mate < 2; ++mate) { const Rec* read = mate ? previous : &record; if (read != nullptr && is_pristine_alignment(*read)) count_viral_read((uint32_t) read->contig); }
				}
			}
		}
		if (!ctx.external_duplicate_marking || !(record.flag & BAMF_DUP)) add_fragment_to_coverage(ctx.coverage, record, coverage_flag, previous, is_read_through);
	}
}


struct Fragment3 { Aln a[3]; uint32_t n; bool single_end, duplicate; };

AGPU_HD bool disjoin_split_read_segments(Aln& split_read, Aln& supplementary) {
	const int min_remaining_supplementary_segment = 10;
	const unsigned int clipped_split_read = split_read.strand ? split_read.preclipping() : split_read.postclipping();
	const unsigned int clipped_supplementary = supplementary.strand ? supplementary.postclipping() : supplementary.preclipping();
	const int overlap = (int) split_read.sequence_length - clipped_split_read - clipped_supplementary;
	if (overlap <= 0) return true;
	const unsigned int clipped_op = supplementary.strand ? supplementary.n_cigar - 1 : 0;
	const unsigned int matching_op = supplementary.strand ? clipped_op - 1 : 1;
	if (supplementary.n_cigar < 2 || (supplementary.cigar(matching_op) & 15) != CIGAR_M || (int) (supplementary.cigar(matching_op) >> 4) < overlap + min_remaining_supplementary_segment) return false;
	const uint32_t clipped_element = supplementary.cigar(clipped_op), matching_element = supplementary.cigar(matching_op);
	supplementary.set_cigar(clipped_op, ((clipped_element >> 4) + overlap) << 4 | (clipped_element & 15));
	supplementary.set_cigar(matching_op, ((matching_element >> 4) - overlap) << 4 | (matching_element & 15));
	if (supplementary.strand) supplementary.end -= overlap; else supplementary.start += overlap;
	return true;
}

AGPU_HD void swap_alignments(Aln& x, Aln& y) { const Aln t = x; x = y; y = t; }
AGPU_HD void take_sequence(Aln& target, const Aln& source) { target.sequence_record = source.sequence_record; target.sequence_length = source.sequence_length; }

AGPU_HD bool normalize_plan(const IngestStream& in, const FragmentPlan& plan, const TandemAlignment* tandem, Fragment3& f) {
	f.single_end = plan.single_end; f.duplicate = plan.duplicate;
	const uint32_t size = plan.count;
	if (size < 2 || size > 3) return false;
	for (uint32_t k = 0; k < size; ++k) f.a[k] = materialize(in, plan.entry[k], tandem);
	for (uint32_t k = 0; k < size; ++k) if (f.a[k].n_cigar == 0) return false;
	Aln* a = f.a;
	f.n = size;
	if (plan.single_end) {
		if (!(size == 2 && (a[MATE1].supplementary != a[MATE2].supplementary))) return false;
		if (a[MATE1].end - a[MATE1].start > a[MATE2].end - a[MATE2].start) { a[2] = a[MATE2]; a[MATE2] = a[MATE1]; }
		else { a[2] = a[MATE1]; a[MATE1] = a[MATE2]; }
		f.n = 3;
		if (!a[MATE1].supplementary) take_sequence(a[SPLIT_READ], a[MATE1]);
		else if (!a[SPLIT_READ].supplementary) take_sequence(a[MATE1], a[SPLIT_READ]);
		else { take_sequence(a[MATE1], a[SUPPLEMENTARY]); take_sequence(a[SPLIT_READ], a[SUPPLEMENTARY]); }
		a[SUPPLEMENTARY].sequence_record = NO_RECORD; a[SUPPLEMENTARY].sequence_length = 0;
		if ((a[MATE1].cigar(0) & 15) == CIGAR_H) a[MATE1].set_cigar(0, a[MATE1].cigar(0) >> 4 << 4 | CIGAR_S);
		if ((a[MATE1].cigar(a[MATE1].n_cigar - 1) & 15) == CIGAR_H) a[MATE1].set_cigar(a[MATE1].n_cigar - 1, a[MATE1].cigar(a[MATE1].n_cigar - 1) >> 4 << 4 | CIGAR_S);
		if ((a[SPLIT_READ].cigar(0) & 15) == CIGAR_H) a[SPLIT_READ].set_cigar(0, a[SPLIT_READ].cigar(0) >> 4 << 4 | CIGAR_S);
		if ((a[SPLIT_READ].cigar(a[SPLIT_READ].n_cigar - 1) & 15) == CIGAR_H) {
			const uint32_t last = a[SPLIT_READ].n_cigar - 1;
			if (last >= a[MATE1].n_cigar) return false;
			a[SPLIT_READ].set_cigar(last, a[MATE1].cigar(last) >> 4 << 4 | CIGAR_S);
		}
		a[SUPPLEMENTARY].supplementary = true; a[MATE1].supplementary = false; a[SPLIT_READ].supplementary = false;
		bool flip_mate1_strand;
		const bool same = a[SPLIT_READ].strand == a[SUPPLEMENTARY].strand;
		const uint64_t length = (uint64_t) (uint32_t) a[SPLIT_READ].sequence_length;
		if (length - a[SPLIT_READ].preclipping() - (same ? a[SUPPLEMENTARY].postclipping() : a[SUPPLEMENTARY].preclipping()) <
		    length - a[SPLIT_READ].postclipping() - (same ? a[SUPPLEMENTARY].preclipping() : a[SUPPLEMENTARY].postclipping()))
			flip_mate1_strand = a[SPLIT_READ].strand == true;
		else
			flip_mate1_strand = a[SPLIT_READ].strand == false;
		a[MATE1].strand = complement_strand_if(a[MATE1].strand, flip_mate1_strand);
		a[SPLIT_READ].strand = complement_strand_if(a[SPLIT_READ].strand, !flip_mate1_strand);
		a[SUPPLEMENTARY].strand = complement_strand_if(a[SUPPLEMENTARY].strand, !flip_mate1_strand);
		a[MATE1].first_in_pair = !flip_mate1_strand;
		a[SPLIT_READ].first_in_pair = flip_mate1_strand;
		a[SUPPLEMENTARY].first_in_pair = flip_mate1_strand;
		if (!disjoin_split_read_segments(a[SPLIT_READ], a[SUPPLEMENTARY])) return false;
	} else {
		if (size == 3) {
			if (a[MATE1].supplementary) swap_alignments(a[MATE1], a[SUPPLEMENTARY]);
			else if (a[MATE2].supplementary) swap_alignments(a[MATE2], a[SUPPLEMENTARY]);
			if (a[SPLIT_READ].first_in_pair != a[SUPPLEMENTARY].first_in_pair) swap_alignments(a[MATE1], a[MATE2]);
			if (a[MATE1].supplementary || a[SPLIT_READ].supplementary || !a[SUPPLEMENTARY].supplementary) return false;
			if (a[MATE1].contig != a[SPLIT_READ].contig || a[MATE1].strand == a[SPLIT_READ].strand) return false;
			if (!disjoin_split_read_segments(a[SPLIT_READ], a[SUPPLEMENTARY])) return false;
		} else {
			if (a[MATE1].supplementary || a[MATE2].supplementary) return false;
		}
	}
	if ((a[MATE1].cigar(0) & 15) == CIGAR_H || (a[MATE1].cigar(a[MATE1].n_cigar - 1) & 15) == CIGAR_H ||
	    (a[MATE2].cigar(0) & 15) == CIGAR_H || (a[MATE2].cigar(a[MATE2].n_cigar - 1) & 15) == CIGAR_H)
		return false;
	return true;
}


AGPU_HD uint32_t decimal_digits(int64_t value, char* out ) {
	char reversed[21]; uint32_t n = 0;
	uint64_t magnitude = value < 0 ? (uint64_t) (-(value + 1)) + 1 : (uint64_t) value;
	do { reversed[n++] = (char) ('0' + magnitude % 10); magnitude /= 10; } while (magnitude > 0);
	uint32_t at = 0;
	if (value < 0) out[at++] = '-';
	while (n > 0) out[at++] = reversed[--n];
	return at;
}

struct FragmentName { const uint8_t* qname; uint32_t qname_length; char suffix[28]; uint32_t suffix_length; };
const uint32_t LENGTH_UNKNOWN = 0xFFFFFFFFu;
AGPU_HD FragmentName fragment_name(const Rec& representative, int64_t hit_index , bool itd, uint32_t length = LENGTH_UNKNOWN ) {
	FragmentName name;
	name.qname = representative.name; name.qname_length = length != LENGTH_UNKNOWN ? length : qname_length(representative);
	name.suffix[0] = ',';
	name.suffix_length = 1 + decimal_digits(hit_index, name.suffix + 1);
	if (itd) { name.suffix[name.suffix_length++] = 'I'; name.suffix[name.suffix_length++] = 'T'; name.suffix[name.suffix_length++] = 'D'; }
	return name;
}
AGPU_HD uint32_t name_length(const FragmentName& name) { return name.qname_length + name.suffix_length; }
AGPU_HD uint8_t name_byte(const FragmentName& name, uint32_t i) { return i < name.qname_length ? name.qname[i] : (i - name.qname_length < name.suffix_length ? (uint8_t) name.suffix[i - name.qname_length] : 0); }
AGPU_HD uint64_t name_chunk(const FragmentName& name, uint32_t chunk) {
	uint64_t value = 0;
	for (uint32_t k = 0; k < 8; ++k) value = value << 8 | name_byte(name, 8 * chunk + k);
	return value;
}
AGPU_HD int compare_names(const FragmentName& x, const FragmentName& y) {
	const uint32_t nx = name_length(x), ny = name_length(y), n = nx < ny ? nx : ny;
	const uint32_t qnames = x.qname_length < y.qname_length ? x.qname_length : y.qname_length, different = first_difference(x.qname, y.qname, qnames);
	if (different < qnames) return x.qname[different] < y.qname[different] ? -1 : 1;
	for (uint32_t i = qnames; i < n; ++i) { const uint8_t cx = name_byte(x, i), cy = name_byte(y, i); if (cx != cy) return cx < cy ? -1 : 1; }
	return nx < ny ? -1 : nx > ny ? 1 : 0;
}


struct FragmentSizes { uint32_t cigar_words, sequence_bytes, name_length; };
AGPU_HD uint32_t padded_sequence_bytes(uint32_t bases) { return (((bases + 1) / 2) + 3) & ~3u; }
AGPU_HD void fragment_sizes(const Fragment3& f, const Rec& representative, int64_t hit_index, bool itd, FragmentSizes& sizes, uint32_t length = LENGTH_UNKNOWN ) {
	uint32_t cigar_words = 0, sequence_bytes = 0;
	for (uint32_t s = 0; s < f.n; ++s) {
		cigar_words += f.a[s].n_cigar;
		if (s < 2) sequence_bytes += padded_sequence_bytes((uint32_t) f.a[s].sequence_length);
	}
	sizes.cigar_words = cigar_words; sizes.sequence_bytes = sequence_bytes;
	sizes.name_length = name_length(fragment_name(representative, hit_index, itd, length));
}

struct PackTarget {
	uint8_t* n_aln; uint8_t* fbits; uint32_t* group;
	uint16_t* contig[3]; int32_t* start[3]; int32_t* end[3]; uint8_t* abits[3]; uint32_t* cigar_offset[3]; uint16_t* cigar_count[3];
	uint32_t* cigar_pool; uint32_t* seq_offset[2]; uint32_t* seq_length[2]; uint8_t* seq_pool; char* names;
	uint64_t* name_offset;
	uint32_t* row_name_offset;
};

AGPU_HD uint32_t write_fragment(const IngestStream& in, const Fragment3& f, const FragmentName& name, uint64_t i, uint64_t cigar_at, uint64_t sequence_at, uint64_t name_at, uint32_t group, const PackTarget& out) {
	out.n_aln[i] = (uint8_t) f.n;
	out.fbits[i] = (f.single_end ? FBIT_SINGLE_END : 0) | (f.duplicate ? FBIT_DUPLICATE : 0);
	out.group[i] = group;
	uint32_t longest = 0;
	for (uint32_t s = 0; s < 3; ++s) {
		if (s >= f.n) {
			out.contig[s][i] = 0; out.start[s][i] = 0; out.end[s][i] = 0; out.abits[s][i] = 0; out.cigar_offset[s][i] = 0; out.cigar_count[s][i] = 0;
			if (s < 2) { out.seq_offset[s][i] = 0; out.seq_length[s][i] = 0; }
			continue;
		}
		const Aln& a = f.a[s];
		out.contig[s][i] = (uint16_t) a.contig; out.start[s][i] = a.start; out.end[s][i] = a.end;
		out.abits[s][i] = (a.strand ? ABIT_STRAND : 0) | (a.first_in_pair ? ABIT_FIRST_IN_PAIR : 0) | (a.supplementary ? ABIT_SUPPLEMENTARY : 0) | ABIT_PREDICTED_STRAND_AMBIGUOUS;
		out.cigar_offset[s][i] = (uint32_t) cigar_at; out.cigar_count[s][i] = (uint16_t) a.n_cigar;
		for (uint32_t k = 0; k < a.n_cigar; ++k) out.cigar_pool[cigar_at + k] = a.cigar(k);
		cigar_at += a.n_cigar;
		if (s < 2) {
			const uint32_t length = (uint32_t) a.sequence_length, bytes = (length + 1) / 2, padded = padded_sequence_bytes(length);
			out.seq_offset[s][i] = (uint32_t) (sequence_at / 4); out.seq_length[s][i] = length;
			if (length > longest) longest = length;
			if (length > 0) {
				const Rec source = load_record(in, a.sequence_record);
				uint32_t* target = (uint32_t*) (out.seq_pool + sequence_at);
				for (uint32_t w = 0; w < padded / 4; ++w) {
					uint32_t value = 0;
					if (4 * w + 4 < bytes) value = load_u32(source.seq_bytes + 4 * w);
					else for (uint32_t b = 0; b < 4; ++b) {
						const uint32_t at = 4 * w + b;
						if (at >= bytes) break;
						uint32_t byte = source.seq_bytes[at];
						if (at == bytes - 1 && (length & 1)) byte &= 0xF0u;
						value |= byte << (8 * b);
					}
					target[w] = value;
				}
			}
			sequence_at += padded;
		}
	}
	out.name_offset[i] = name_at;
	const uint32_t length = name_length(name);
	uint32_t copied = 0;
	for (; copied + 8 <= name.qname_length; copied += 8) { const uint64_t word = load_u64(name.qname + copied); __builtin_memcpy(out.names + name_at + copied, &word, 8); }
	for (uint32_t k = copied; k < name.qname_length; ++k) out.names[name_at + k] = (char) name.qname[k];
	for (uint32_t k = name.qname_length; k < length; ++k) out.names[name_at + k] = (char) name_byte(name, k);
	return longest;
}

AGPU_HD void row_sizes(const BatchView& b, const uint64_t* name_offset, uint64_t i, uint32_t& cigar_words, uint32_t& sequence_bytes, uint32_t& name_bytes) {
	cigar_words = 0; sequence_bytes = 0;
	for (uint32_t s = 0; s < b.n_aln[i]; ++s) {
		cigar_words += b.cigar_count[s][i];
		if (s < 2) sequence_bytes += padded_sequence_bytes(b.seq_length[s][i]);
	}
	name_bytes = name_offset ? (uint32_t) (name_offset[i + 1] - name_offset[i]) : 0;
}
AGPU_HD void copy_row(const BatchView& b, const uint8_t* pristine_fbits, const uint8_t* const* pristine_abits, const uint64_t* name_offset, const char* names, uint64_t i, uint64_t k,
                      uint64_t cigar_at, uint64_t sequence_at, uint64_t name_at, const PackTarget& out) {
	const uint32_t n_aln = b.n_aln[i];
	out.n_aln[k] = (uint8_t) n_aln; out.fbits[k] = pristine_fbits[i]; out.group[k] = b.group[i];
	for (uint32_t s = 0; s < 3; ++s) {
		out.contig[s][k] = b.contig[s][i]; out.start[s][k] = b.start[s][i]; out.end[s][k] = b.end[s][i]; out.abits[s][k] = pristine_abits[s][i];
		const uint32_t count = s < n_aln ? b.cigar_count[s][i] : 0;
		out.cigar_count[s][k] = (uint16_t) count; out.cigar_offset[s][k] = s < n_aln ? (uint32_t) cigar_at : 0;
		for (uint32_t c = 0; c < count; ++c) out.cigar_pool[cigar_at + c] = b.cigar_pool[b.cigar_offset[s][i] + c];
		cigar_at += count;
		if (s < 2) {
			const uint32_t length = s < n_aln ? b.seq_length[s][i] : 0, padded = padded_sequence_bytes(length);
			out.seq_length[s][k] = length; out.seq_offset[s][k] = s < n_aln ? (uint32_t) (sequence_at / 4) : 0;
			if (length > 0) {
				const uint32_t* source = (const uint32_t*) b.seq_pool + b.seq_offset[s][i];
				uint32_t* target = (uint32_t*) (out.seq_pool + sequence_at);
				for (uint32_t w = 0; w < padded / 4; ++w) target[w] = source[w];
			}
			sequence_at += padded;
		}
	}
	if (out.name_offset) out.name_offset[k] = name_at; else out.row_name_offset[k] = (uint32_t) name_at;
	if (name_offset) for (uint64_t c = name_offset[i]; c < name_offset[i + 1]; ++c) out.names[name_at + (c - name_offset[i])] = names[c];
}

AGPU_HD uint8_t strandedness_vote(const BatchView& b, const AnnotationView& ann, uint64_t i) {
	if (b.n_aln[i] != 3) return 0;
	const bool split_strand = b.abits[SPLIT_READ][i] & ABIT_STRAND, supplementary_strand = b.abits[SUPPLEMENTARY][i] & ABIT_STRAND;
	int32_t distance = b.start[SPLIT_READ][i] - b.start[SUPPLEMENTARY][i]; if (distance < 0) distance = -distance;
	if (!(b.contig[SPLIT_READ][i] == b.contig[SUPPLEMENTARY][i] && split_strand == supplementary_strand && distance < 400000)) return 0;
	AGPU_IDSET(genes);
	query_by_coordinate(ann.gene_index, b.contig[SPLIT_READ][i], b.start[SPLIT_READ][i], b.end[SPLIT_READ][i], IdentityMap(), genes);
	if (genes.n != 1 || genes.overflow) return 0;
	const uint32_t gene = genes.get(0);
	const int32_t position = split_strand ? b.start[SPLIT_READ][i] : b.end[SPLIT_READ][i];
	if (!is_breakpoint_spliced(ann, gene, split_strand, position)) return 0;
	const bool gene_strand = ann.gene_bits[gene] & GBIT_STRAND, mate1_strand = b.abits[MATE1][i] & ABIT_STRAND;
	const bool matching = ((b.abits[SPLIT_READ][i] & ABIT_FIRST_IN_PAIR) && split_strand == gene_strand) || ((b.abits[MATE1][i] & ABIT_FIRST_IN_PAIR) && mate1_strand == gene_strand);
	return matching ? 3 : 1;
}

}

#endif
```

Before: 60.77 million.

## Slim alignment summaries, keep replay plans in LDS, and cut private-memory indexing

After: 60.21 million. About the same (-0.9%).

```diff
diff --git a/arriba_amd/csrc/device/agpu_ingest.hip b/arriba_amd/csrc/device/agpu_ingest.hip
--- a/arriba_amd/csrc/device/agpu_ingest.hip
+++ b/arriba_amd/csrc/device/agpu_ingest.hip
@@ -262,6 +262,8 @@
 template <bool RUNS> __global__ void __launch_bounds__(BLOCK) AGPU_REPLAY_OCCUPANCY group_replay_kernel(IngestContext ctx, const uint32_t* sorted_records, const uint32_t* group_begin, const uint32_t* group_count, uint32_t first_group, uint32_t n_groups,
                                                              FragmentPlan* plain, TandemPlan* itd, uint8_t* valid, FragmentSizes* sizes, unsigned long long* viral_counts, uint32_t* qname_differs, uint32_t* counters) {
 	__shared__ uint32_t sums[2];
+	__shared__ FragmentPlan plain_plans[BLOCK];
+	__shared__ TandemPlan itd_plans[BLOCK];
 	GroupTally tally; tally.malformed = 0; tally.chimeric = 0; tally.collision = 0;
 	const uint32_t g = first_group + blockIdx.x * BLOCK + threadIdx.x;
 	if (g < n_groups) {
@@ -284,16 +286,17 @@
 				if (unsorted) atomicOr(&counters[IC_RUNS_UNSORTED], 1u);
 			}
 		}
-		FragmentPlan plain_plan; TandemPlan itd_plan;
+		FragmentPlan& plain_plan = plain_plans[threadIdx.x]; TandemPlan& itd_plan = itd_plans[threadIdx.x];
 		ViralCounter viral = { viral_counts };
 		replay_group(ctx, sorted_records + begin, n_records, plain_plan, itd_plan, tally, viral, RUNS ? &representative : nullptr, length, hit);
 		if (tally.collision) atomicOr(&counters[IC_COLLISION], 1u);
 		Fragment3 fragment;
 		AGPU_NOUNROLL for (uint32_t entry = 0; entry < 2; ++entry) {
-			const FragmentPlan& plan = entry ? itd_plan.plan : plain_plan;
+			FragmentPlan plan = plain_plan;
+			if (entry) plan = itd_plan.plan;
 			bool ok = false;
 			if (plan.count > 0) {
-				ok = normalize_plan(ctx.stream, plan, entry ? &itd_plan.tandem : nullptr, fragment);
+				ok = normalize_plan(ctx.stream, plan, &itd_plan.tandem, fragment);
 				if (!ok) tally.malformed++;
 			}
 			valid[2 * (size_t) g + entry] = ok;
@@ -307,7 +310,7 @@
 }
 
 
-__device__ FragmentName name_of(const IngestStream& in, const uint32_t* group_first, uint32_t ref, Rec& storage) {
+__device__ __forceinline__ FragmentName name_of(const IngestStream& in, const uint32_t* group_first, uint32_t ref, Rec& storage) {
 	storage = load_record(in, group_first[ref >> 1]);
 	return fragment_name(storage, hit_index_of(in, group_first[ref >> 1], storage), ref & 1);
 }
@@ -378,9 +381,9 @@
 		const bool is_itd = ref & 1;
 		Fragment3 f;
 		normalize_plan(in, is_itd ? itd[g].plan : plain[g], is_itd ? &itd[g].tandem : nullptr, f);
+		atomicMax(&block_max, write_alignments(in, f, i, cigar_base[i], sequence_base[i], group_id[i], out));
 		Rec storage;
-		const FragmentName name = name_of(in, group_first, ref, storage);
-		atomicMax(&block_max, write_fragment(in, f, name, i, cigar_base[i], sequence_base[i], name_base[i], group_id[i], out));
+		write_name(name_of(in, group_first, ref, storage), i, name_base[i], out);
 	}
 	__syncthreads();
 	if (threadIdx.x == 0 && block_max) atomicMax(&counters[IC_MAX_READ_LENGTH], block_max);
diff --git a/arriba_amd/csrc/device/ingest_core.hpp b/arriba_amd/csrc/device/ingest_core.hpp
--- a/arriba_amd/csrc/device/ingest_core.hpp
+++ b/arriba_amd/csrc/device/ingest_core.hpp
@@ -255,88 +255,93 @@
 struct TandemPlan { FragmentPlan plan; TandemAlignment tandem; };
 
 AGPU_HD void plan_clear(FragmentPlan& plan) { plan.count = 0; plan.single_end = 0; plan.duplicate = 0; plan.reserved = 0; for (int k = 0; k < 3; ++k) { plan.entry[k].record = NO_RECORD; plan.entry[k].cigar_index = 0; plan.entry[k].clip = 0; plan.entry[k].supplementary = 0; } }
+AGPU_HD void plan_store(FragmentPlan& plan, const PlanEntry& e) {
+	if (plan.count == 0) plan.entry[0] = e; else if (plan.count == 1) plan.entry[1] = e; else if (plan.count == 2) plan.entry[2] = e;
+	if (plan.count < 255) ++plan.count;
+}
 AGPU_HD void plan_push(FragmentPlan& plan, uint32_t record, const Rec& r, bool is_supplementary, uint32_t cigar_index, uint8_t clip) {
 	plan.single_end = !(r.flag & BAMF_PAIRED);
 	plan.duplicate = plan.duplicate || (r.flag & BAMF_DUP);
-	if (plan.count < 3) {
-		PlanEntry& e = plan.entry[plan.count];
-		e.record = record; e.cigar_index = (uint16_t) cigar_index; e.clip = clip; e.supplementary = is_supplementary;
-	}
-	if (plan.count < 255) ++plan.count;
+	PlanEntry e; e.record = record; e.cigar_index = (uint16_t) cigar_index; e.clip = clip; e.supplementary = is_supplementary;
+	plan_store(plan, e);
 }
 AGPU_HD void plan_push_tandem(FragmentPlan& plan) {
-	if (plan.count < 3) { PlanEntry& e = plan.entry[plan.count]; e.record = NO_RECORD; e.cigar_index = 0; e.clip = PLAN_TANDEM; e.supplementary = 0; }
-	if (plan.count < 255) ++plan.count;
-}
-
-struct Aln {
-	const uint8_t* cigar_bytes;
-	uint32_t record;
+	PlanEntry e; e.record = NO_RECORD; e.cigar_index = 0; e.clip = PLAN_TANDEM; e.supplementary = 0;
+	plan_store(plan, e);
+}
+
+template <class T> AGPU_HD T pick(bool condition, T yes, T no) { return condition ? yes : no; }
+
+struct AlnSummary {
+	uint64_t cigar_at;
+	uint32_t front0, front1, back1, back0;
+	uint32_t n_cigar;
 	uint32_t sequence_record;
 	int32_t sequence_length;
 	int32_t contig, start, end;
-	uint32_t n_cigar;
-	uint32_t cigar_index;
-	uint32_t patch_index[2], patch_value[2];
-	uint32_t tandem_cigar[3];
-	uint32_t made_index, made_value, shift;
-	uint8_t clip, n_patch;
-	bool supplementary, first_in_pair, strand;
-	AGPU_HD uint32_t base_cigar(uint32_t i) const {
-		if (clip == PLAN_TANDEM) return i == 0 ? tandem_cigar[0] : i == 1 ? tandem_cigar[1] : tandem_cigar[2];
-		if (i == made_index) return made_value;
-		return load_u32(cigar_bytes + 4 * (size_t) (i + shift));
-	}
-	AGPU_HD uint32_t cigar(uint32_t i) const {
-		uint32_t value = base_cigar(i);
-		for (uint32_t k = 0; k < n_patch; ++k) if (patch_index[k] == i) value = patch_value[k];
-		return value;
-	}
-	AGPU_HD void set_cigar(uint32_t i, uint32_t value) {
-		for (uint32_t k = 0; k < n_patch; ++k) if (patch_index[k] == i) { patch_value[k] = value; return; }
-		if (n_patch < 2) { patch_index[n_patch] = i; patch_value[n_patch] = value; ++n_patch; }
-	}
-	AGPU_HD uint32_t preclipping() const { const uint32_t c = cigar(0), op = c & 15; return (op == CIGAR_S || op == CIGAR_H) ? c >> 4 : 0; }
-	AGPU_HD uint32_t postclipping() const { const uint32_t c = cigar(n_cigar - 1), op = c & 15; return (op == CIGAR_S || op == CIGAR_H) ? c >> 4 : 0; }
+	uint32_t bits;
+	AGPU_HD bool supplementary() const { return bits & ABIT_SUPPLEMENTARY; }
+	AGPU_HD bool first_in_pair() const { return bits & ABIT_FIRST_IN_PAIR; }
+	AGPU_HD bool strand() const { return bits & ABIT_STRAND; }
+	AGPU_HD void set_bit(uint32_t bit, bool value) { bits = value ? bits | bit : bits & ~bit; }
+	AGPU_HD bool is_edge(uint32_t i) const { return i < 2 || i + 2 >= n_cigar; }
+	AGPU_HD uint32_t edge(uint32_t i) const { return pick(i == 0, front0, pick(i == 1, front1, pick(i + 1 == n_cigar, back0, back1))); }
+	AGPU_HD void set_edge(uint32_t i, uint32_t value) { if (i == 0) front0 = value; if (i == 1) front1 = value; if (i + 2 == n_cigar) back1 = value; if (i + 1 == n_cigar) back0 = value; }
+	AGPU_HD uint32_t cigar(const IngestStream& in, uint32_t i) const { return is_edge(i) ? edge(i) : load_u32(in.bytes + cigar_at + 4 * (uint64_t) i); }
+	AGPU_HD uint32_t preclipping() const { const uint32_t op = front0 & 15; return (op == CIGAR_S || op == CIGAR_H) ? front0 >> 4 : 0; }
+	AGPU_HD uint32_t postclipping() const { const uint32_t op = back0 & 15; return (op == CIGAR_S || op == CIGAR_H) ? back0 >> 4 : 0; }
 };
 
-AGPU_HD Aln materialize(const IngestStream& in, const PlanEntry& e, const TandemAlignment* tandem) {
-	Aln a;
-	a.n_patch = 0; a.patch_index[0] = a.patch_index[1] = 0; a.patch_value[0] = a.patch_value[1] = 0;
-	a.tandem_cigar[0] = a.tandem_cigar[1] = a.tandem_cigar[2] = 0;
-	a.clip = e.clip; a.cigar_index = e.cigar_index;
-	a.made_index = NO_RECORD; a.made_value = 0; a.shift = 0;
+AGPU_HD AlnSummary empty_summary() {
+	AlnSummary a;
+	a.cigar_at = 0; a.front0 = a.front1 = a.back1 = a.back0 = 0; a.n_cigar = 0; a.sequence_record = NO_RECORD; a.sequence_length = 0;
+	a.contig = 0; a.start = 0; a.end = 0; a.bits = 0;
+	return a;
+}
+
+AGPU_HD uint32_t record_edge(const Rec& r, uint32_t i, uint32_t n, uint32_t shift, uint32_t made_index) {
+	const uint32_t source = i + shift;
+	return (i < n && i != made_index && source < r.n_cigar) ? r.cigar(source) : 0u;
+}
+
+AGPU_HD AlnSummary summarize(const IngestStream& in, const PlanEntry& e, const TandemAlignment* tandem) {
+	AlnSummary a = empty_summary();
 	if (e.clip == PLAN_TANDEM) {
 		const Rec source = load_record(in, tandem->record);
-		a.cigar_bytes = source.cigar_bytes;
-		a.record = NO_RECORD;
-		a.supplementary = tandem->supplementary; a.first_in_pair = tandem->first_in_pair; a.strand = tandem->strand;
+		a.bits = (tandem->supplementary ? ABIT_SUPPLEMENTARY : 0) | (tandem->first_in_pair ? ABIT_FIRST_IN_PAIR : 0) | (tandem->strand ? ABIT_STRAND : 0);
 		a.contig = source.contig; a.start = tandem->start; a.end = tandem->end;
-		a.n_cigar = tandem->n_cigar;
-		for (int k = 0; k < 3; ++k) a.tandem_cigar[k] = tandem->cigar[k];
-		a.sequence_record = a.supplementary ? NO_RECORD : tandem->record;
-		a.sequence_length = a.supplementary ? 0 : source.l_seq;
+		const uint32_t n = tandem->n_cigar, c0 = tandem->cigar[0], c1 = tandem->cigar[1], c2 = tandem->cigar[2];
+		a.n_cigar = n;
+		a.front0 = c0; a.front1 = c1;
+		a.back0 = n == 1 ? c0 : n == 2 ? c1 : c2;
+		a.back1 = n == 2 ? c0 : n == 3 ? c1 : 0;
+		a.sequence_record = a.supplementary() ? NO_RECORD : tandem->record;
+		a.sequence_length = a.supplementary() ? 0 : source.l_seq;
 		return a;
 	}
 	const Rec r = load_record(in, e.record);
-	a.cigar_bytes = r.cigar_bytes;
-	a.record = e.record;
-	a.strand = r.forward(); a.first_in_pair = r.flag & BAMF_READ1; a.contig = r.contig; a.supplementary = e.supplementary;
+	a.bits = (r.forward() ? ABIT_STRAND : 0) | ((r.flag & BAMF_READ1) ? ABIT_FIRST_IN_PAIR : 0) | (e.supplementary ? ABIT_SUPPLEMENTARY : 0); a.contig = r.contig;
+	uint32_t shift = 0;
 	a.sequence_record = e.supplementary ? NO_RECORD : e.record;
 	a.sequence_length = e.supplementary ? 0 : r.l_seq;
+	uint32_t made_index = NO_RECORD, made_value = 0;
 	if (e.clip == CLIP_START) {
 		a.start = r.pos + r.rlen(e.cigar_index); a.end = r.endpos() - 1;
 		a.n_cigar = r.n_cigar - e.cigar_index + 1;
-		a.made_index = 0; a.made_value = (uint32_t) r.qlen(e.cigar_index) << 4 | (r.op(0) == CIGAR_H ? CIGAR_H : CIGAR_S);
-		a.shift = (uint32_t) e.cigar_index - 1u;
+		made_index = 0; made_value = (uint32_t) r.qlen(e.cigar_index) << 4 | (r.op(0) == CIGAR_H ? CIGAR_H : CIGAR_S);
+		shift = (uint32_t) e.cigar_index - 1u;
 	} else if (e.clip == CLIP_END) {
 		a.start = r.pos; a.end = r.pos + r.rlen((uint32_t) e.cigar_index + 1) - 1;
 		a.n_cigar = (uint32_t) e.cigar_index + 2;
-		a.made_index = (uint32_t) e.cigar_index + 1; a.made_value = (uint32_t) (r.l_seq - r.qlen((uint32_t) e.cigar_index + 1)) << 4 | (r.op(r.n_cigar - 1) == CIGAR_H ? CIGAR_H : CIGAR_S);
+		made_index = (uint32_t) e.cigar_index + 1; made_value = (uint32_t) (r.l_seq - r.qlen((uint32_t) e.cigar_index + 1)) << 4 | (r.op(r.n_cigar - 1) == CIGAR_H ? CIGAR_H : CIGAR_S);
 	} else {
 		a.start = r.pos; a.end = r.endpos() - 1;
 		a.n_cigar = r.n_cigar;
 	}
+	const uint32_t n = a.n_cigar;
+	a.cigar_at = (uint64_t) (r.cigar_bytes - in.bytes) + 4 * (uint64_t) (int64_t) (int32_t) shift;
+	a.front0 = record_edge(r, 0u, n, shift, made_index); a.front1 = record_edge(r, 1u, n, shift, made_index); a.back1 = record_edge(r, n - 2u, n, shift, made_index); a.back0 = record_edge(r, n - 1u, n, shift, made_index);
+	if (made_index != NO_RECORD) a.set_edge(made_index, made_value);
 	return a;
 }
 
@@ -479,11 +484,11 @@
 			uint32_t clip_right = clipped_start ? r->l_seq - clipped_length : 0;
 			if (tandem_start > contig_pos) clip_left += tandem_start - contig_pos;
 			if (tandem_end < contig_pos + (int) clipped_length - 1) clip_right += contig_pos + clipped_length - 1 - tandem_end;
-			tandem.n_cigar = 0;
-			tandem.cigar[0] = tandem.cigar[1] = tandem.cigar[2] = 0;
-			if (clip_left > 0) tandem.cigar[tandem.n_cigar++] = clip_left << 4 | CIGAR_S;
-			tandem.cigar[tandem.n_cigar++] = (uint32_t) (tandem_end - tandem_start + 1) << 4 | CIGAR_M;
-			if (clip_right > 0) tandem.cigar[tandem.n_cigar++] = clip_right << 4 | CIGAR_S;
+			const uint32_t left = clip_left << 4 | CIGAR_S, match = (uint32_t) (tandem_end - tandem_start + 1) << 4 | CIGAR_M, right = clip_right << 4 | CIGAR_S;
+			tandem.cigar[0] = clip_left > 0 ? left : match;
+			tandem.cigar[1] = clip_left > 0 ? match : clip_right > 0 ? right : 0;
+			tandem.cigar[2] = clip_left > 0 && clip_right > 0 ? right : 0;
+			tandem.n_cigar = (uint8_t) (1 + (clip_left > 0) + (clip_right > 0));
 			return true;
 		}
 	}
@@ -742,109 +747,141 @@
 }
 
 
-struct Fragment3 { Aln a[3]; uint32_t n; bool single_end, duplicate; };
-
-AGPU_HD bool disjoin_split_read_segments(Aln& split_read, Aln& supplementary) {
+struct Fragment3 { AlnSummary a[3]; uint32_t n; bool single_end, duplicate; };
+
+AGPU_HD bool disjoin_split_read_segments(const AlnSummary& split_read, AlnSummary& supplementary) {
 	const int min_remaining_supplementary_segment = 10;
-	const unsigned int clipped_split_read = split_read.strand ? split_read.preclipping() : split_read.postclipping();
-	const unsigned int clipped_supplementary = supplementary.strand ? supplementary.postclipping() : supplementary.preclipping();
+	const unsigned int clipped_split_read = split_read.strand() ? split_read.preclipping() : split_read.postclipping();
+	const unsigned int clipped_supplementary = supplementary.strand() ? supplementary.postclipping() : supplementary.preclipping();
 	const int overlap = (int) split_read.sequence_length - clipped_split_read - clipped_supplementary;
 	if (overlap <= 0) return true;
-	const unsigned int clipped_op = supplementary.strand ? supplementary.n_cigar - 1 : 0;
-	const unsigned int matching_op = supplementary.strand ? clipped_op - 1 : 1;
-	if (supplementary.n_cigar < 2 || (supplementary.cigar(matching_op) & 15) != CIGAR_M || (int) (supplementary.cigar(matching_op) >> 4) < overlap + min_remaining_supplementary_segment) return false;
-	const uint32_t clipped_element = supplementary.cigar(clipped_op), matching_element = supplementary.cigar(matching_op);
-	supplementary.set_cigar(clipped_op, ((clipped_element >> 4) + overlap) << 4 | (clipped_element & 15));
-	supplementary.set_cigar(matching_op, ((matching_element >> 4) - overlap) << 4 | (matching_element & 15));
-	if (supplementary.strand) supplementary.end -= overlap; else supplementary.start += overlap;
+	if (supplementary.n_cigar < 2) return false;
+	const uint32_t clipped_element = pick(supplementary.strand(), supplementary.back0, supplementary.front0), matching_element = pick(supplementary.strand(), supplementary.back1, supplementary.front1);
+	if ((matching_element & 15) != CIGAR_M || (int) (matching_element >> 4) < overlap + min_remaining_supplementary_segment) return false;
+	const uint32_t clipped_op = supplementary.strand() ? supplementary.n_cigar - 1 : 0, matching_op = supplementary.strand() ? clipped_op - 1 : 1;
+	supplementary.set_edge(clipped_op, ((clipped_element >> 4) + overlap) << 4 | (clipped_element & 15));
+	supplementary.set_edge(matching_op, ((matching_element >> 4) - overlap) << 4 | (matching_element & 15));
+	if (supplementary.strand()) supplementary.end -= overlap; else supplementary.start += overlap;
 	return true;
 }
 
-AGPU_HD void swap_alignments(Aln& x, Aln& y) { const Aln t = x; x = y; y = t; }
-AGPU_HD void take_sequence(Aln& target, const Aln& source) { target.sequence_record = source.sequence_record; target.sequence_length = source.sequence_length; }
+template <class T> AGPU_HD void swap_values(T& x, T& y) { const T t = x; x = y; y = t; }
+AGPU_HD AlnSummary pick_summary(bool condition, const AlnSummary& yes, const AlnSummary& no) {
+	AlnSummary a;
+	a.cigar_at = pick(condition, yes.cigar_at, no.cigar_at); a.bits = pick(condition, yes.bits, no.bits);
+	a.front0 = pick(condition, yes.front0, no.front0); a.front1 = pick(condition, yes.front1, no.front1); a.back1 = pick(condition, yes.back1, no.back1); a.back0 = pick(condition, yes.back0, no.back0);
+	a.n_cigar = pick(condition, yes.n_cigar, no.n_cigar); a.sequence_record = pick(condition, yes.sequence_record, no.sequence_record); a.sequence_length = pick(condition, yes.sequence_length, no.sequence_length);
+	a.contig = pick(condition, yes.contig, no.contig); a.start = pick(condition, yes.start, no.start); a.end = pick(condition, yes.end, no.end);
+	return a;
+}
+AGPU_HD PlanEntry plan_entry(const FragmentPlan& plan, uint32_t k) {
+	uint64_t words[3];
+	for (int e = 0; e < 3; ++e) __builtin_memcpy(&words[e], &plan.entry[e], 8);
+	const uint64_t word = pick(k == 0, words[0], pick(k == 1, words[1], words[2]));
+	PlanEntry entry;
+	__builtin_memcpy(&entry, &word, 8);
+	return entry;
+}
+static_assert(sizeof(PlanEntry) == 8, "plan_entry copies a PlanEntry as one word");
+struct EntryFlags { bool supplementary, first_in_pair; };
+AGPU_HD EntryFlags entry_flags(const IngestStream& in, const PlanEntry& e, const TandemAlignment* tandem) {
+	EntryFlags flags;
+	if (e.clip == PLAN_TANDEM) { flags.supplementary = tandem->supplementary; flags.first_in_pair = tandem->first_in_pair; }
+	else { flags.supplementary = e.supplementary; flags.first_in_pair = load_u16(in.bytes + in.record_offset[e.record] + 4 + 14) & BAMF_READ1; }
+	return flags;
+}
+AGPU_HD void take_sequence(AlnSummary& target, const AlnSummary& source) { target.sequence_record = source.sequence_record; target.sequence_length = source.sequence_length; }
+AGPU_HD void soften_front(AlnSummary& a) { if ((a.front0 & 15) == CIGAR_H) a.set_edge(0, a.front0 >> 4 << 4 | CIGAR_S); }
+AGPU_HD bool hard_clipped(const AlnSummary& a) { return (a.front0 & 15) == CIGAR_H || (a.back0 & 15) == CIGAR_H; }
 
 AGPU_HD bool normalize_plan(const IngestStream& in, const FragmentPlan& plan, const TandemAlignment* tandem, Fragment3& f) {
 	f.single_end = plan.single_end; f.duplicate = plan.duplicate;
 	const uint32_t size = plan.count;
+	f.n = size;
+	AlnSummary& mate1 = f.a[MATE1]; AlnSummary& mate2 = f.a[MATE2]; AlnSummary& third = f.a[SUPPLEMENTARY];
+	mate1 = empty_summary(); mate2 = empty_summary(); third = empty_summary();
 	if (size < 2 || size > 3) return false;
-	for (uint32_t k = 0; k < size; ++k) f.a[k] = materialize(in, plan.entry[k], tandem);
-	for (uint32_t k = 0; k < size; ++k) if (f.a[k].n_cigar == 0) return false;
-	Aln* a = f.a;
-	f.n = size;
+	uint32_t entry_of_mate1 = 0, entry_of_mate2 = 1, entry_of_third = 2;
+	if (!plan.single_end && size == 3) {
+		EntryFlags flags1 = entry_flags(in, plan.entry[0], tandem), flags2 = entry_flags(in, plan.entry[1], tandem), flags3 = entry_flags(in, plan.entry[2], tandem);
+		if (flags1.supplementary) { swap_values(flags1, flags3); swap_values(entry_of_mate1, entry_of_third); }
+		else if (flags2.supplementary) { swap_values(flags2, flags3); swap_values(entry_of_mate2, entry_of_third); }
+		if (flags2.first_in_pair != flags3.first_in_pair) { swap_values(flags1, flags2); swap_values(entry_of_mate1, entry_of_mate2); }
+	}
+	mate1 = summarize(in, plan_entry(plan, entry_of_mate1), tandem);
+	mate2 = summarize(in, plan_entry(plan, entry_of_mate2), tandem);
+	if (size == 3) third = summarize(in, plan_entry(plan, entry_of_third), tandem);
+	if (mate1.n_cigar == 0 || mate2.n_cigar == 0 || (size == 3 && third.n_cigar == 0)) return false;
 	if (plan.single_end) {
-		if (!(size == 2 && (a[MATE1].supplementary != a[MATE2].supplementary))) return false;
-		if (a[MATE1].end - a[MATE1].start > a[MATE2].end - a[MATE2].start) { a[2] = a[MATE2]; a[MATE2] = a[MATE1]; }
-		else { a[2] = a[MATE1]; a[MATE1] = a[MATE2]; }
+		if (!(size == 2 && (mate1.supplementary() != mate2.supplementary()))) return false;
+		const bool first_is_longer = mate1.end - mate1.start > mate2.end - mate2.start;
+		const AlnSummary longer = pick_summary(first_is_longer, mate1, mate2);
+		third = pick_summary(first_is_longer, mate2, mate1);
+		mate1 = longer; mate2 = longer;
 		f.n = 3;
-		if (!a[MATE1].supplementary) take_sequence(a[SPLIT_READ], a[MATE1]);
-		else if (!a[SPLIT_READ].supplementary) take_sequence(a[MATE1], a[SPLIT_READ]);
-		else { take_sequence(a[MATE1], a[SUPPLEMENTARY]); take_sequence(a[SPLIT_READ], a[SUPPLEMENTARY]); }
-		a[SUPPLEMENTARY].sequence_record = NO_RECORD; a[SUPPLEMENTARY].sequence_length = 0;
-		if ((a[MATE1].cigar(0) & 15) == CIGAR_H) a[MATE1].set_cigar(0, a[MATE1].cigar(0) >> 4 << 4 | CIGAR_S);
-		if ((a[MATE1].cigar(a[MATE1].n_cigar - 1) & 15) == CIGAR_H) a[MATE1].set_cigar(a[MATE1].n_cigar - 1, a[MATE1].cigar(a[MATE1].n_cigar - 1) >> 4 << 4 | CIGAR_S);
-		if ((a[SPLIT_READ].cigar(0) & 15) == CIGAR_H) a[SPLIT_READ].set_cigar(0, a[SPLIT_READ].cigar(0) >> 4 << 4 | CIGAR_S);
-		if ((a[SPLIT_READ].cigar(a[SPLIT_READ].n_cigar - 1) & 15) == CIGAR_H) {
-			const uint32_t last = a[SPLIT_READ].n_cigar - 1;
-			if (last >= a[MATE1].n_cigar) return false;
-			a[SPLIT_READ].set_cigar(last, a[MATE1].cigar(last) >> 4 << 4 | CIGAR_S);
-		}
-		a[SUPPLEMENTARY].supplementary = true; a[MATE1].supplementary = false; a[SPLIT_READ].supplementary = false;
+		if (!mate1.supplementary()) take_sequence(mate2, mate1);
+		else if (!mate2.supplementary()) take_sequence(mate1, mate2);
+		else { take_sequence(mate1, third); take_sequence(mate2, third); }
+		third.sequence_record = NO_RECORD; third.sequence_length = 0;
+		soften_front(mate1);
+		if ((mate1.back0 & 15) == CIGAR_H) mate1.set_edge(mate1.n_cigar - 1, mate1.back0 >> 4 << 4 | CIGAR_S);
+		soften_front(mate2);
+		if ((mate2.back0 & 15) == CIGAR_H) {
+			const uint32_t last = mate2.n_cigar - 1;
+			if (last >= mate1.n_cigar) return false;
+			mate2.set_edge(last, mate1.cigar(in, last) >> 4 << 4 | CIGAR_S);
+		}
+		third.set_bit(ABIT_SUPPLEMENTARY, true); mate1.set_bit(ABIT_SUPPLEMENTARY, false); mate2.set_bit(ABIT_SUPPLEMENTARY, false);
 		bool flip_mate1_strand;
-		const bool same = a[SPLIT_READ].strand == a[SUPPLEMENTARY].strand;
-		const uint64_t length = (uint64_t) (uint32_t) a[SPLIT_READ].sequence_length;
-		if (length - a[SPLIT_READ].preclipping() - (same ? a[SUPPLEMENTARY].postclipping() : a[SUPPLEMENTARY].preclipping()) <
-		    length - a[SPLIT_READ].postclipping() - (same ? a[SUPPLEMENTARY].preclipping() : a[SUPPLEMENTARY].postclipping()))
-			flip_mate1_strand = a[SPLIT_READ].strand == true;
+		const bool same = mate2.strand() == third.strand();
+		const uint64_t length = (uint64_t) (uint32_t) mate2.sequence_length;
+		if (length - mate2.preclipping() - (same ? third.postclipping() : third.preclipping()) <
+		    length - mate2.postclipping() - (same ? third.preclipping() : third.postclipping()))
+			flip_mate1_strand = mate2.strand() == true;
 		else
-			flip_mate1_strand = a[SPLIT_READ].strand == false;
-		a[MATE1].strand = complement_strand_if(a[MATE1].strand, flip_mate1_strand);
-		a[SPLIT_READ].strand = complement_strand_if(a[SPLIT_READ].strand, !flip_mate1_strand);
-		a[SUPPLEMENTARY].strand = complement_strand_if(a[SUPPLEMENTARY].strand, !flip_mate1_strand);
-		a[MATE1].first_in_pair = !flip_mate1_strand;
-		a[SPLIT_READ].first_in_pair = flip_mate1_strand;
-		a[SUPPLEMENTARY].first_in_pair = flip_mate1_strand;
-		if (!disjoin_split_read_segments(a[SPLIT_READ], a[SUPPLEMENTARY])) return false;
+			flip_mate1_strand = mate2.strand() == false;
+		mate1.set_bit(ABIT_STRAND, complement_strand_if(mate1.strand(), flip_mate1_strand));
+		mate2.set_bit(ABIT_STRAND, complement_strand_if(mate2.strand(), !flip_mate1_strand));
+		third.set_bit(ABIT_STRAND, complement_strand_if(third.strand(), !flip_mate1_strand));
+		mate1.set_bit(ABIT_FIRST_IN_PAIR, !flip_mate1_strand);
+		mate2.set_bit(ABIT_FIRST_IN_PAIR, flip_mate1_strand);
+		third.set_bit(ABIT_FIRST_IN_PAIR, flip_mate1_strand);
+		if (!disjoin_split_read_segments(mate2, third)) return false;
 	} else {
 		if (size == 3) {
-			if (a[MATE1].supplementary) swap_alignments(a[MATE1], a[SUPPLEMENTARY]);
-			else if (a[MATE2].supplementary) swap_alignments(a[MATE2], a[SUPPLEMENTARY]);
-			if (a[SPLIT_READ].first_in_pair != a[SUPPLEMENTARY].first_in_pair) swap_alignments(a[MATE1], a[MATE2]);
-			if (a[MATE1].supplementary || a[SPLIT_READ].supplementary || !a[SUPPLEMENTARY].supplementary) return false;
-			if (a[MATE1].contig != a[SPLIT_READ].contig || a[MATE1].strand == a[SPLIT_READ].strand) return false;
-			if (!disjoin_split_read_segments(a[SPLIT_READ], a[SUPPLEMENTARY])) return false;
+			if (mate1.supplementary() || mate2.supplementary() || !third.supplementary()) return false;
+			if (mate1.contig != mate2.contig || mate1.strand() == mate2.strand()) return false;
+			if (!disjoin_split_read_segments(mate2, third)) return false;
 		} else {
-			if (a[MATE1].supplementary || a[MATE2].supplementary) return false;
-		}
-	}
-	if ((a[MATE1].cigar(0) & 15) == CIGAR_H || (a[MATE1].cigar(a[MATE1].n_cigar - 1) & 15) == CIGAR_H ||
-	    (a[MATE2].cigar(0) & 15) == CIGAR_H || (a[MATE2].cigar(a[MATE2].n_cigar - 1) & 15) == CIGAR_H)
-		return false;
+			if (mate1.supplementary() || mate2.supplementary()) return false;
+		}
+	}
+	if (hard_clipped(mate1) || hard_clipped(mate2)) return false;
 	return true;
 }
 
 
-AGPU_HD uint32_t decimal_digits(int64_t value, char* out ) {
-	char reversed[21]; uint32_t n = 0;
-	uint64_t magnitude = value < 0 ? (uint64_t) (-(value + 1)) + 1 : (uint64_t) value;
-	do { reversed[n++] = (char) ('0' + magnitude % 10); magnitude /= 10; } while (magnitude > 0);
-	uint32_t at = 0;
-	if (value < 0) out[at++] = '-';
-	while (n > 0) out[at++] = reversed[--n];
-	return at;
-}
-
-struct FragmentName { const uint8_t* qname; uint32_t qname_length; char suffix[28]; uint32_t suffix_length; };
+struct FragmentName { const uint8_t* qname; uint32_t qname_length; uint32_t suffix_length; uint64_t suffix0, suffix1, suffix2; };
 const uint32_t LENGTH_UNKNOWN = 0xFFFFFFFFu;
+AGPU_HD void suffix_prepend(FragmentName& name, char c) {
+	name.suffix2 = name.suffix2 << 8 | name.suffix1 >> 56; name.suffix1 = name.suffix1 << 8 | name.suffix0 >> 56; name.suffix0 = name.suffix0 << 8 | (uint8_t) c;
+	++name.suffix_length;
+}
 AGPU_HD FragmentName fragment_name(const Rec& representative, int64_t hit_index , bool itd, uint32_t length = LENGTH_UNKNOWN ) {
 	FragmentName name;
 	name.qname = representative.name; name.qname_length = length != LENGTH_UNKNOWN ? length : qname_length(representative);
-	name.suffix[0] = ',';
-	name.suffix_length = 1 + decimal_digits(hit_index, name.suffix + 1);
-	if (itd) { name.suffix[name.suffix_length++] = 'I'; name.suffix[name.suffix_length++] = 'T'; name.suffix[name.suffix_length++] = 'D'; }
+	name.suffix0 = itd ? 0x445449ull  : 0; name.suffix1 = 0; name.suffix2 = 0; name.suffix_length = itd ? 3 : 0;
+	uint64_t magnitude = hit_index < 0 ? (uint64_t) (-(hit_index + 1)) + 1 : (uint64_t) hit_index;
+	while (magnitude >> 32) { suffix_prepend(name, (char) ('0' + magnitude % 10)); magnitude /= 10; }
+	uint32_t low = (uint32_t) magnitude;
+	do { suffix_prepend(name, (char) ('0' + low % 10)); low /= 10; } while (low > 0);
+	if (hit_index < 0) suffix_prepend(name, '-');
+	suffix_prepend(name, ',');
 	return name;
 }
 AGPU_HD uint32_t name_length(const FragmentName& name) { return name.qname_length + name.suffix_length; }
-AGPU_HD uint8_t name_byte(const FragmentName& name, uint32_t i) { return i < name.qname_length ? name.qname[i] : (i - name.qname_length < name.suffix_length ? (uint8_t) name.suffix[i - name.qname_length] : 0); }
+AGPU_HD uint8_t suffix_byte(const FragmentName& name, uint32_t k) { return k >= 24 ? 0 : (uint8_t) (pick(k < 8, name.suffix0, pick(k < 16, name.suffix1, name.suffix2)) >> (8 * (k & 7))); }
+AGPU_HD uint8_t name_byte(const FragmentName& name, uint32_t i) { return i < name.qname_length ? name.qname[i] : suffix_byte(name, i - name.qname_length); }
 AGPU_HD uint64_t name_chunk(const FragmentName& name, uint32_t chunk) {
 	uint64_t value = 0;
 	for (uint32_t k = 0; k < 8; ++k) value = value << 8 | name_byte(name, 8 * chunk + k);
@@ -862,11 +899,8 @@
 struct FragmentSizes { uint32_t cigar_words, sequence_bytes, name_length; };
 AGPU_HD uint32_t padded_sequence_bytes(uint32_t bases) { return (((bases + 1) / 2) + 3) & ~3u; }
 AGPU_HD void fragment_sizes(const Fragment3& f, const Rec& representative, int64_t hit_index, bool itd, FragmentSizes& sizes, uint32_t length = LENGTH_UNKNOWN ) {
-	uint32_t cigar_words = 0, sequence_bytes = 0;
-	for (uint32_t s = 0; s < f.n; ++s) {
-		cigar_words += f.a[s].n_cigar;
-		if (s < 2) sequence_bytes += padded_sequence_bytes((uint32_t) f.a[s].sequence_length);
-	}
+	uint32_t cigar_words = f.a[0].n_cigar + f.a[1].n_cigar, sequence_bytes = padded_sequence_bytes((uint32_t) f.a[0].sequence_length) + padded_sequence_bytes((uint32_t) f.a[1].sequence_length);
+	if (f.n > 2) cigar_words += f.a[2].n_cigar;
 	sizes.cigar_words = cigar_words; sizes.sequence_bytes = sequence_bytes;
 	sizes.name_length = name_length(fragment_name(representative, hit_index, itd, length));
 }
@@ -879,52 +913,69 @@
 	uint32_t* row_name_offset;
 };
 
-AGPU_HD uint32_t write_fragment(const IngestStream& in, const Fragment3& f, const FragmentName& name, uint64_t i, uint64_t cigar_at, uint64_t sequence_at, uint64_t name_at, uint32_t group, const PackTarget& out) {
+template <uint32_t S> AGPU_HD uint32_t write_slot(const IngestStream& in, const Fragment3& f, uint64_t i, uint64_t& cigar_at, uint64_t& sequence_at, const PackTarget& out) {
+	if (S >= f.n) {
+		out.contig[S][i] = 0; out.start[S][i] = 0; out.end[S][i] = 0; out.abits[S][i] = 0; out.cigar_offset[S][i] = 0; out.cigar_count[S][i] = 0;
+		if constexpr (S < 2) { out.seq_offset[S][i] = 0; out.seq_length[S][i] = 0; }
+		return 0;
+	}
+	const AlnSummary& a = f.a[S];
+	out.contig[S][i] = (uint16_t) a.contig; out.start[S][i] = a.start; out.end[S][i] = a.end;
+	out.abits[S][i] = (uint8_t) (a.bits | ABIT_PREDICTED_STRAND_AMBIGUOUS);
+	out.cigar_offset[S][i] = (uint32_t) cigar_at; out.cigar_count[S][i] = (uint16_t) a.n_cigar;
+	const uint32_t n = a.n_cigar;
+	uint32_t* cigar = out.cigar_pool + cigar_at;
+	if (n > 0) cigar[0] = a.front0;
+	if (n > 1) cigar[1] = a.front1;
+	if (n > 4) { const uint8_t* middle = in.bytes + a.cigar_at; for (uint32_t k = 2; k + 2 < n; ++k) cigar[k] = load_u32(middle + 4 * (uint64_t) k); }
+	if (n > 3) cigar[n - 2] = a.back1;
+	if (n > 2) cigar[n - 1] = a.back0;
+	cigar_at += n;
+	uint32_t length = 0;
+	if constexpr (S < 2) {
+		length = (uint32_t) a.sequence_length;
+		const uint32_t bytes = (length + 1) / 2, padded = padded_sequence_bytes(length);
+		out.seq_offset[S][i] = (uint32_t) (sequence_at / 4); out.seq_length[S][i] = length;
+		if (length > 0) {
+			const Rec source = load_record(in, a.sequence_record);
+			uint32_t* target = (uint32_t*) (out.seq_pool + sequence_at);
+			for (uint32_t w = 0; w < padded / 4; ++w) {
+				uint32_t value = 0;
+				if (4 * w + 4 < bytes) value = load_u32(source.seq_bytes + 4 * w);
+				else for (uint32_t b = 0; b < 4; ++b) {
+					const uint32_t at = 4 * w + b;
+					if (at >= bytes) break;
+					uint32_t byte = source.seq_bytes[at];
+					if (at == bytes - 1 && (length & 1)) byte &= 0xF0u;
+					value |= byte << (8 * b);
+				}
+				target[w] = value;
+			}
+		}
+		sequence_at += padded;
+	}
+	return length;
+}
+
+AGPU_HD uint32_t write_alignments(const IngestStream& in, const Fragment3& f, uint64_t i, uint64_t cigar_at, uint64_t sequence_at, uint32_t group, const PackTarget& out) {
 	out.n_aln[i] = (uint8_t) f.n;
 	out.fbits[i] = (f.single_end ? FBIT_SINGLE_END : 0) | (f.duplicate ? FBIT_DUPLICATE : 0);
 	out.group[i] = group;
-	uint32_t longest = 0;
-	for (uint32_t s = 0; s < 3; ++s) {
-		if (s >= f.n) {
-			out.contig[s][i] = 0; out.start[s][i] = 0; out.end[s][i] = 0; out.abits[s][i] = 0; out.cigar_offset[s][i] = 0; out.cigar_count[s][i] = 0;
-			if (s < 2) { out.seq_offset[s][i] = 0; out.seq_length[s][i] = 0; }
-			continue;
-		}
-		const Aln& a = f.a[s];
-		out.contig[s][i] = (uint16_t) a.contig; out.start[s][i] = a.start; out.end[s][i] = a.end;
-		out.abits[s][i] = (a.strand ? ABIT_STRAND : 0) | (a.first_in_pair ? ABIT_FIRST_IN_PAIR : 0) | (a.supplementary ? ABIT_SUPPLEMENTARY : 0) | ABIT_PREDICTED_STRAND_AMBIGUOUS;
-		out.cigar_offset[s][i] = (uint32_t) cigar_at; out.cigar_count[s][i] = (uint16_t) a.n_cigar;
-		for (uint32_t k = 0; k < a.n_cigar; ++k) out.cigar_pool[cigar_at + k] = a.cigar(k);
-		cigar_at += a.n_cigar;
-		if (s < 2) {
-			const uint32_t length = (uint32_t) a.sequence_length, bytes = (length + 1) / 2, padded = padded_sequence_bytes(length);
-			out.seq_offset[s][i] = (uint32_t) (sequence_at / 4); out.seq_length[s][i] = length;
-			if (length > longest) longest = length;
-			if (length > 0) {
-				const Rec source = load_record(in, a.sequence_record);
-				uint32_t* target = (uint32_t*) (out.seq_pool + sequence_at);
-				for (uint32_t w = 0; w < padded / 4; ++w) {
-					uint32_t value = 0;
-					if (4 * w + 4 < bytes) value = load_u32(source.seq_bytes + 4 * w);
-					else for (uint32_t b = 0; b < 4; ++b) {
-						const uint32_t at = 4 * w + b;
-						if (at >= bytes) break;
-						uint32_t byte = source.seq_bytes[at];
-						if (at == bytes - 1 && (length & 1)) byte &= 0xF0u;
-						value |= byte << (8 * b);
-					}
-					target[w] = value;
-				}
-			}
-			sequence_at += padded;
-		}
-	}
+	const uint32_t length0 = write_slot<0>(in, f, i, cigar_at, sequence_at, out), length1 = write_slot<1>(in, f, i, cigar_at, sequence_at, out);
+	write_slot<2>(in, f, i, cigar_at, sequence_at, out);
+	return length0 > length1 ? length0 : length1;
+}
+AGPU_HD void write_name(const FragmentName& name, uint64_t i, uint64_t name_at, const PackTarget& out) {
 	out.name_offset[i] = name_at;
 	const uint32_t length = name_length(name);
 	uint32_t copied = 0;
 	for (; copied + 8 <= name.qname_length; copied += 8) { const uint64_t word = load_u64(name.qname + copied); __builtin_memcpy(out.names + name_at + copied, &word, 8); }
 	for (uint32_t k = copied; k < name.qname_length; ++k) out.names[name_at + k] = (char) name.qname[k];
 	for (uint32_t k = name.qname_length; k < length; ++k) out.names[name_at + k] = (char) name_byte(name, k);
+}
+AGPU_HD uint32_t write_fragment(const IngestStream& in, const Fragment3& f, const FragmentName& name, uint64_t i, uint64_t cigar_at, uint64_t sequence_at, uint64_t name_at, uint32_t group, const PackTarget& out) {
+	const uint32_t longest = write_alignments(in, f, i, cigar_at, sequence_at, group, out);
+	write_name(name, i, name_at, out);
 	return longest;
 }
 
```
